# tangle-network/zk-SaaS

Hardware: AMD Instinct MI355X
Metric: Groth16 proofs/sec (SHA-256 circuit) (higher is better)
Workload: dtype u32 limbs (256-bit Montgomery); 1 GPU; BASELINE configs[3]: full distributed Groth16 on the SHA-256 circuit, BN254, l=2, n=8 parties on one GPU, all 12 masks sampled and applied (sha256.rs:226-291); masks=True, constraints=30006, wires=29823, domain=32768, len_a=14911, len_w=14911, len_u=16384, parties=8, packing_factor=2, fixed_base_tables=True

## Files before the change

include/zksaas.h:

```cpp
#ifndef ZKSAAS_H
#define ZKSAAS_H

#include <stddef.h>
#include <stdint.h>

#ifdef __cplusplus
extern "C" {
#endif

typedef struct zk_ctx zk_ctx;

enum zk_curve { ZK_BN254 = 0, ZK_BLS12_381 = 1, ZK_BLS12_377 = 2 };
enum zk_group { ZK_G1 = 1, ZK_G2 = 2 };
enum zk_status { ZK_OK = 0, ZK_ERR_GENERIC = 1, ZK_ERR_PROTOCOL = 2, ZK_ERR_NOT_CONNECTED = 3, ZK_ERR_BAD_INPUT = 4 };

int zk_ctx_create(int curve, int l, int device, zk_ctx** out);
void zk_ctx_destroy(zk_ctx* ctx);
const char* zk_last_error(zk_ctx* ctx, int* party);
int zk_ctx_n(const zk_ctx* ctx);
int zk_ctx_l(const zk_ctx* ctx);
size_t zk_fr_bytes(const zk_ctx* ctx);
size_t zk_fq_bytes(const zk_ctx* ctx);
const char* zk_version(void);

int zk_malloc(zk_ctx* ctx, size_t bytes, void** out_d);
int zk_free(zk_ctx* ctx, void* p_d);
int zk_memcpy_h2d(zk_ctx* ctx, void* dst_d, const void* src, size_t bytes, void* stream);
int zk_memcpy_d2h(zk_ctx* ctx, void* dst, const void* src_d, size_t bytes, void* stream);
int zk_stream_sync(zk_ctx* ctx, void* stream);

void zk_chacha20_block(const uint32_t key[8], uint64_t counter, uint64_t nonce, uint32_t out[16]);

int zk_pss_pack(zk_ctx* ctx, const void* secrets_d, size_t nchunks, int order, uint64_t seed, void* shares_d,
                void* stream);
int zk_pss_det_pack(zk_ctx* ctx, const void* secrets_d, size_t nchunks, int order, void* shares_d,
                    void* stream);
int zk_pss_unpack(zk_ctx* ctx, const void* shares_d, size_t nchunks, void* secrets_d, void* stream);
int zk_pss_unpack2(zk_ctx* ctx, const void* shares_d, const uint32_t* parties, int nparties, size_t nchunks,
                   void* secrets_d, void* stream);

int zk_bitrev(zk_ctx* ctx, void* x_d, int log2_len, void* stream);
int zk_vec_add(zk_ctx* ctx, void* x_d, const void* y_d, size_t len, void* stream);
int zk_vec_scale(zk_ctx* ctx, void* x_d, const void* k, size_t len, void* stream);
int zk_vec_mul_sub(zk_ctx* ctx, void* out_d, const void* a_d, const void* b_d, const void* c_d, size_t len,
                   void* stream);

int zk_fft1(zk_ctx* ctx, void* shares_d, int log2_m, int inverse, size_t batch, const void* add_d, void* stream);
int zk_fq_selftest(zk_ctx* ctx, int op, const void* a_d, const void* b_d, const void* c_d, const void* d_d, size_t len,
                   void* out_d, void* stream);
int zk_fft2_king(zk_ctx* ctx, const void* in_d, const uint32_t* parties, int nparties, int log2_m, int inverse,
                 const void* g, int scale_size_inv, int rearrange, uint64_t seed, void* out_d,
                 const void* out_mask_d, void* stream);
int zk_d_fft(zk_ctx* ctx, void* shares_d, const void* in_mask_d, const void* out_mask_d, int rearrange,
             int log2_m, uint64_t seed, void* out_d, void* stream);
int zk_d_ifft(zk_ctx* ctx, void* shares_d, const void* in_mask_d, const void* out_mask_d, int rearrange,
              int log2_m, const void* g, uint64_t seed, void* out_d, void* stream);
int zk_fft_mask_sample(zk_ctx* ctx, int rearrange, const void* g, int inverse, int log2_m, uint64_t seed,
                       void* in_mask_d, void* out_mask_d, void* stream);

int zk_deg_red(zk_ctx* ctx, void* x_d, const void* in_mask_d, const void* out_mask_d, size_t len, uint64_t seed,
               void* stream);
int zk_deg_red_parties(zk_ctx* ctx, const void* x_d, const uint32_t* parties, int nparties, const void* in_mask_d,
                       const void* out_mask_d, size_t len, uint64_t seed, void* out_d, void* stream);
int zk_degred_mask_sample(zk_ctx* ctx, size_t len, uint64_t seed, void* in_mask_d, void* out_mask_d,
                          void* stream);
int zk_d_pp(zk_ctx* ctx, const void* num_d, const void* den_d, const void* in_mask_d, const void* out_mask_d,
            size_t len, uint64_t seed, void* out_d, void* stream);

int zk_deg_red_points(zk_ctx* ctx, int group, const void* x_d, const void* in_mask_d, const void* out_mask_d, size_t len,
                      const void* gen_affine, uint64_t seed, void* out_d, void* stream);
int zk_degred_mask_sample_points(zk_ctx* ctx, int group, const void* gen_affine, size_t len, uint64_t seed,
                                 void* in_mask_d, void* out_mask_d, void* stream);

int zk_msm(zk_ctx* ctx, int group, const void* bases_d, size_t len_bases, const void* scalars_d,
           size_t len_scalars, void* out, void* stream);
int zk_d_msm(zk_ctx* ctx, int group, const void* bases_d, const void* scalars_d, size_t len, const void* in_mask,
             const void* out_mask, void* out, void* stream);

int zk_pss_pack_points(zk_ctx* ctx, int group, const void* points_d, size_t nchunks, int points_per_chunk,
                       void* shares_d, void* stream);
int zk_base_mul(zk_ctx* ctx, int group, const void* base_affine, const void* scalars_d, size_t len,
                void* out_affine_d, void* stream);

typedef struct zk_groth16_masks {
  const void* fft_in[6];
  const void* fft_out[6];
  const void* degred_in;
  const void* degred_out;
  const void* msm_in[5];
  const void* msm_out[5];
} zk_groth16_masks;

typedef struct zk_crs_share {
  const void* s_d;
  const void* h_d;
  const void* v_d;
  const void* w_d;
  const void* u_d;
  size_t len_a, len_w, len_u;
  const void *a_query0, *b_g1_query0, *delta_g1, *alpha_g1, *beta_g1;
  const void *b_g2_query0, *delta_g2, *beta_g2;
} zk_crs_share;

int zk_circom_h(zk_ctx* ctx, const void* qap_a_d, const void* qap_b_d, const void* qap_c_d, int log2_m,
                const zk_groth16_masks* masks, uint64_t seed, void* h_d, void* stream);
int zk_groth16_prove(zk_ctx* ctx, const zk_crs_share* crs, const void* qap_a_d, const void* qap_b_d,
                     const void* qap_c_d, const void* a_share_d, const void* ax_share_d, const void* r, const void* s,
                     int log2_m, const zk_groth16_masks* masks, uint64_t seed, void* pi_a, void* pi_b, void* pi_c,
                     void* stream);

int zk_d_msm_local(zk_ctx* ctx, int group, const void* bases_d, const void* scalars_d, size_t len, int first_party,
                   int nparties, const void* in_mask, void* out, void* stream);
int zk_group_add(zk_ctx* ctx, int group, const void* a, const void* b, void* out);
int zk_msm_plan(zk_ctx* ctx, int group, size_t len, int plan[4]);
int zk_msm_precompute(zk_ctx* ctx, int group, const void* bases_d, size_t len, void* stream);
int zk_msm_forget(zk_ctx* ctx, const void* bases_d);
int zk_msm_table_info(zk_ctx* ctx, int group, const void* bases_d, int info[2]);
int zk_ctx_set_option(zk_ctx* ctx, const char* name, long long value);
int zk_msm_mask_sample(zk_ctx* ctx, int group, const void* gen_affine, uint64_t seed, void* in_mask, void* out_mask);

int zk_r1cs_qap(zk_ctx* ctx, const void* a_row_ptr_d, const void* a_col_d, const void* a_val_d,
                const void* b_row_ptr_d, const void* b_col_d, const void* b_val_d, const void* w_d,
                size_t num_variables, size_t num_constraints, size_t num_instance, int log_m, void* a_out_d,
                void* b_out_d, void* c_out_d, void* stream);
int zk_fr_to_bytes(zk_ctx* ctx, const void* x_d, size_t len, void* bytes_out_d, void* stream);
int zk_fr_from_bytes(zk_ctx* ctx, const void* bytes_d, size_t len, void* x_out_d, void* stream);
int zk_points_decompress(zk_ctx* ctx, int group, const void* bytes_d, size_t len, void* out_affine_d, void* stream);
int zk_points_compress(zk_ctx* ctx, int group, const void* affine_d, size_t len, void* bytes_out_d, void* stream);
int zk_libsnark_h(zk_ctx* ctx, const void* qap_a_d, const void* qap_b_d, const void* qap_c_d, int log2_m,
                  const void* const* fft_in, const void* const* fft_out, uint64_t seed, void* h_d, void* stream);
int zk_groth16_msms_begin(zk_ctx* ctx, const zk_crs_share* crs, const void* a_share_d, const void* ax_share_d,
                          int first_party, int nparties, int skip_h, const zk_groth16_masks* masks, void* stream);
int zk_groth16_msms_finish(zk_ctx* ctx, const void* h_share_d, void* const* out, void* stream);
int zk_groth16_prove_async(zk_ctx* ctx, const zk_crs_share* crs, const void* qap_a_d, const void* qap_b_d,
                           const void* qap_c_d, const void* a_share_d, const void* ax_share_d, const void* r,
                           const void* s, int log2_m, const zk_groth16_masks* masks, uint64_t seed, void* stream,
                           int* handle);
int zk_groth16_wait(zk_ctx* ctx, int handle, void* pi_a, void* pi_b, void* pi_c);
int zk_groth16_abort(zk_ctx* ctx, int handle);
int zk_groth16_assemble(zk_ctx* ctx, const zk_crs_share* crs, const void* r, const void* s, const void* const* sums,
                        const zk_groth16_masks* masks, void* pi_a, void* pi_b, void* pi_c);
int zk_groth16_prove_batch(zk_ctx* ctx, const zk_crs_share* crs, int nproofs, const void* const* qap_a_d,
                           const void* const* qap_b_d, const void* const* qap_c_d, const void* const* a_share_d,
                           const void* const* ax_share_d, const void* r, const void* s, int log2_m,
                           const zk_groth16_masks* masks, uint64_t seed, void* pi_a, void* pi_b, void* pi_c, void* stream);
int zk_groth16_prove_batch_async(zk_ctx* ctx, const zk_crs_share* crs, int nproofs, const void* const* qap_a_d,
                                 const void* const* qap_b_d, const void* const* qap_c_d, const void* const* a_share_d,
                                 const void* const* ax_share_d, const void* r, const void* s, int log2_m,
                                 const zk_groth16_masks* masks, uint64_t seed, void* stream, int* handle);
int zk_groth16_batch_wait(zk_ctx* ctx, int handle, void* pi_a, void* pi_b, void* pi_c);
int zk_msm_batch(zk_ctx* ctx, int group, const void* bases_d, size_t len, const void* const* scalars_d, int nvec,
                 void* out, void* stream);
int zk_pss_unpack_points(zk_ctx* ctx, int group, const void* shares_d, size_t nchunks, void* out_d, void* stream);
int zk_pss_unpack2_points(zk_ctx* ctx, int group, const void* shares_d, const uint32_t* parties, int nparties,
                          size_t nchunks, void* out_d, void* stream);
int zk_groth16_reconstruct(zk_ctx* ctx, const void* pi_a, const void* pi_b, const void* pi_c, const uint32_t* parties,
                           int nparties, void* proof_affine, void* proof_bytes, void* stream);

typedef struct zk_net zk_net;
enum zk_transport { ZK_NET_LOCAL = 0, ZK_NET_RCCL = 1, ZK_NET_SHM = 2 };
#define ZK_NET_ID_BYTES 512
int zk_net_unique_id(void* id_out);
int zk_net_create(zk_ctx* ctx, int transport, int rank, int world, int n_parties ,
                  const int* party_to_rank, const void* id, size_t shm_bytes_per_channel, zk_net** out);
void zk_net_destroy(zk_net* net);
const char* zk_net_last_error(zk_net* net, int* party);
int zk_net_set_timeout_ms(zk_net* net, uint64_t ms);
int zk_net_info(const zk_net* net, int info[4]);
int zk_net_parties(const zk_net* net, int rank, int* parties );
int zk_net_stats(const zk_net* net, uint64_t stats[4]);
int zk_net_enter(zk_net* net, int sid, uint32_t* mask);
int zk_net_gather(zk_net* net, int sid, uint32_t mask, const void* local, size_t bytes_per_rank, void* full);
int zk_net_scatter(zk_net* net, int sid, uint32_t mask, const void* full, size_t bytes_per_rank, void* local);
int zk_net_alltoall(zk_net* net, int sid, uint32_t mask, const void* send, size_t bytes_per_peer, void* recv);
int zk_net_gather_host(zk_net* net, int sid, uint32_t mask, const void* mine, size_t bytes, void* all);
int zk_net_bcast_host(zk_net* net, int sid, uint32_t mask, void* buf, size_t bytes);
int zk_net_sync(zk_net* net, int sid);

int zk_dist_d_fft(zk_ctx* ctx, zk_net* net, int sid, void* shares_d, const void* in_mask_d, const void* out_mask_d,
                  int rearrange, int log2_m, uint64_t seed, void* stream);
int zk_dist_d_ifft(zk_ctx* ctx, zk_net* net, int sid, void* shares_d, const void* in_mask_d, const void* out_mask_d,
                   int rearrange, int log2_m, const void* g, uint64_t seed, void* stream);
int zk_dist_deg_red(zk_ctx* ctx, zk_net* net, int sid, void* x_d, const void* in_mask_d, const void* out_mask_d,
                    size_t len, uint64_t seed, void* stream);
int zk_dist_d_pp(zk_ctx* ctx, zk_net* net, int sid, const void* num_d, const void* den_d, const void* in_mask_d,
                 const void* out_mask_d, size_t len, uint64_t seed, void* out_d, void* stream);
int zk_dist_d_msm(zk_ctx* ctx, zk_net* net, int sid, int group, const void* bases_d, const void* scalars_d, size_t len,
                  const void* in_mask, const void* out_mask, void* out, void* stream);
int zk_dist_deg_red_points(zk_ctx* ctx, zk_net* net, int sid, int group, const void* x_d, const void* in_mask_d,
                           const void* out_mask_d, size_t len, const void* gen_affine, uint64_t seed, void* out_d,
                           void* stream);
int zk_dist_libsnark_h(zk_ctx* ctx, zk_net* net, const void* qap_a_d, const void* qap_b_d, const void* qap_c_d, int log2_m,
                       const void* const* fft_in_masks, const void* const* fft_out_masks, uint64_t seed, void* h_d,
                       void* stream);
int zk_dist_circom_h(zk_ctx* ctx, zk_net* net, const void* qap_a_d, const void* qap_b_d, const void* qap_c_d, int log2_m,
                     const zk_groth16_masks* masks, uint64_t seed, void* h_d, void* stream);
int zk_dist_groth16_prove(zk_ctx* ctx, zk_net* net, const zk_crs_share* crs, const void* qap_a_d, const void* qap_b_d,
                          const void* qap_c_d, const void* a_share_d, const void* ax_share_d, const void* r, const void* s,
                          int log2_m, const zk_groth16_masks* masks, uint64_t seed, void* pi_a, void* pi_b, void* pi_c,
                          void* stream);

int zk_dist_groth16_prove_async(zk_ctx* ctx, zk_net* net, const zk_crs_share* crs, const void* qap_a_d, const void* qap_b_d,
// ... 41 lines not shown
```

rust/zksaas-hip-sys/src/lib.rs:

```rust
#![allow(non_camel_case_types, non_snake_case, clippy::too_many_arguments)]
use core::ffi::{c_char, c_int, c_long, c_longlong, c_void};

pub const ZK_NET_ID_BYTES: usize = 512;

pub const ZK_BN254: c_int = 0;
pub const ZK_BLS12_381: c_int = 1;
pub const ZK_BLS12_377: c_int = 2;

pub const ZK_G1: c_int = 1;
pub const ZK_G2: c_int = 2;

pub const ZK_OK: c_int = 0;
pub const ZK_ERR_GENERIC: c_int = 1;
pub const ZK_ERR_PROTOCOL: c_int = 2;
pub const ZK_ERR_NOT_CONNECTED: c_int = 3;
pub const ZK_ERR_BAD_INPUT: c_int = 4;

pub const ZK_NET_LOCAL: c_int = 0;
pub const ZK_NET_RCCL: c_int = 1;
pub const ZK_NET_SHM: c_int = 2;

#[repr(C)]
pub struct ZkCtx {
    _private: [u8; 0],
}
#[repr(C)]
pub struct ZkNet {
    _private: [u8; 0],
}

#[repr(C)]
#[derive(Clone, Copy)]
pub struct ZkGroth16Masks {
    pub fft_in: [*const c_void; 6],
    pub fft_out: [*const c_void; 6],
    pub degred_in: *const c_void,
    pub degred_out: *const c_void,
    pub msm_in: [*const c_void; 5],
    pub msm_out: [*const c_void; 5],
}

#[repr(C)]
#[derive(Clone, Copy)]
pub struct ZkCrsShare {
    pub s_d: *const c_void,
    pub h_d: *const c_void,
    pub v_d: *const c_void,
    pub w_d: *const c_void,
    pub u_d: *const c_void,
    pub len_a: usize,
    pub len_w: usize,
    pub len_u: usize,
    pub a_query0: *const c_void,
    pub b_g1_query0: *const c_void,
    pub delta_g1: *const c_void,
    pub alpha_g1: *const c_void,
    pub beta_g1: *const c_void,
    pub b_g2_query0: *const c_void,
    pub delta_g2: *const c_void,
    pub beta_g2: *const c_void,
}

#[link(name = "zksaas_hip")]
extern "C" {
    pub fn zk_ctx_create(curve: c_int, l: c_int, device: c_int, out: *mut *mut ZkCtx) -> c_int;
    pub fn zk_ctx_destroy(ctx: *mut ZkCtx);
    pub fn zk_last_error(ctx: *mut ZkCtx, party: *mut c_int) -> *const c_char;
    pub fn zk_ctx_n(ctx: *const ZkCtx) -> c_int;
    pub fn zk_ctx_l(ctx: *const ZkCtx) -> c_int;
    pub fn zk_fr_bytes(ctx: *const ZkCtx) -> usize;
    pub fn zk_fq_bytes(ctx: *const ZkCtx) -> usize;
    pub fn zk_version() -> *const c_char;
    pub fn zk_malloc(ctx: *mut ZkCtx, bytes: usize, out_d: *mut *mut c_void) -> c_int;
    pub fn zk_free(ctx: *mut ZkCtx, p_d: *mut c_void) -> c_int;
    pub fn zk_memcpy_h2d(
        ctx: *mut ZkCtx,
        dst_d: *mut c_void,
        src: *const c_void,
        bytes: usize,
        stream: *mut c_void,
    ) -> c_int;
    pub fn zk_memcpy_d2h(
        ctx: *mut ZkCtx,
        dst: *mut c_void,
        src_d: *const c_void,
        bytes: usize,
        stream: *mut c_void,
    ) -> c_int;
    pub fn zk_stream_sync(ctx: *mut ZkCtx, stream: *mut c_void) -> c_int;
    pub fn zk_chacha20_block(key: *const u32 , counter: u64, nonce: u64, out: *mut u32 );
    pub fn zk_pss_pack(
        ctx: *mut ZkCtx,
        secrets_d: *const c_void,
        nchunks: usize,
        order: c_int,
        seed: u64,
        shares_d: *mut c_void,
        stream: *mut c_void,
    ) -> c_int;
    pub fn zk_pss_det_pack(
        ctx: *mut ZkCtx,
        secrets_d: *const c_void,
        nchunks: usize,
        order: c_int,
        shares_d: *mut c_void,
        stream: *mut c_void,
    ) -> c_int;
    pub fn zk_pss_unpack(
        ctx: *mut ZkCtx,
        shares_d: *const c_void,
        nchunks: usize,
        secrets_d: *mut c_void,
        stream: *mut c_void,
    ) -> c_int;
    pub fn zk_pss_unpack2(
        ctx: *mut ZkCtx,
        shares_d: *const c_void,
        parties: *const u32,
        nparties: c_int,
        nchunks: usize,
        secrets_d: *mut c_void,
        stream: *mut c_void,
    ) -> c_int;
    pub fn zk_bitrev(ctx: *mut ZkCtx, x_d: *mut c_void, log2_len: c_int, stream: *mut c_void) -> c_int;
    pub fn zk_vec_add(
        ctx: *mut ZkCtx,
        x_d: *mut c_void,
        y_d: *const c_void,
        len: usize,
        stream: *mut c_void,
    ) -> c_int;
    pub fn zk_vec_scale(
        ctx: *mut ZkCtx,
        x_d: *mut c_void,
        k: *const c_void,
        len: usize,
        stream: *mut c_void,
    ) -> c_int;
    pub fn zk_vec_mul_sub(
        ctx: *mut ZkCtx,
        out_d: *mut c_void,
        a_d: *const c_void,
        b_d: *const c_void,
        c_d: *const c_void,
        len: usize,
        stream: *mut c_void,
    ) -> c_int;
    pub fn zk_fft1(
        ctx: *mut ZkCtx,
        shares_d: *mut c_void,
        log2_m: c_int,
        inverse: c_int,
        batch: usize,
        add_d: *const c_void,
        stream: *mut c_void,
    ) -> c_int;
    pub fn zk_fq_selftest(
        ctx: *mut ZkCtx,
        op: c_int,
        a_d: *const c_void,
        b_d: *const c_void,
        c_d: *const c_void,
        d_d: *const c_void,
        len: usize,
        out_d: *mut c_void,
        stream: *mut c_void,
    ) -> c_int;
    pub fn zk_fft2_king(
        ctx: *mut ZkCtx,
        in_d: *const c_void,
        parties: *const u32,
        nparties: c_int,
        log2_m: c_int,
        inverse: c_int,
        g: *const c_void,
        scale_size_inv: c_int,
        rearrange: c_int,
        seed: u64,
        out_d: *mut c_void,
        out_mask_d: *const c_void,
        stream: *mut c_void,
    ) -> c_int;
    pub fn zk_d_fft(
        ctx: *mut ZkCtx,
        shares_d: *mut c_void,
        in_mask_d: *const c_void,
        out_mask_d: *const c_void,
        rearrange: c_int,
        log2_m: c_int,
        seed: u64,
        out_d: *mut c_void,
        stream: *mut c_void,
    ) -> c_int;
    pub fn zk_d_ifft(
        ctx: *mut ZkCtx,
        shares_d: *mut c_void,
        in_mask_d: *const c_void,
        out_mask_d: *const c_void,
        rearrange: c_int,
        log2_m: c_int,
        g: *const c_void,
        seed: u64,
        out_d: *mut c_void,
        stream: *mut c_void,
    ) -> c_int;
    pub fn zk_fft_mask_sample(
        ctx: *mut ZkCtx,
        rearrange: c_int,
        g: *const c_void,
        inverse: c_int,
        log2_m: c_int,
        seed: u64,
        in_mask_d: *mut c_void,
        out_mask_d: *mut c_void,
        stream: *mut c_void,
    ) -> c_int;
    pub fn zk_deg_red(
        ctx: *mut ZkCtx,
        x_d: *mut c_void,
        in_mask_d: *const c_void,
        out_mask_d: *const c_void,
        len: usize,
        seed: u64,
        stream: *mut c_void,
    ) -> c_int;
    pub fn zk_deg_red_parties(
        ctx: *mut ZkCtx,
        x_d: *const c_void,
        parties: *const u32,
        nparties: c_int,
        in_mask_d: *const c_void,
        out_mask_d: *const c_void,
        len: usize,
        seed: u64,
        out_d: *mut c_void,
        stream: *mut c_void,
    ) -> c_int;
    pub fn zk_degred_mask_sample(
        ctx: *mut ZkCtx,
        len: usize,
        seed: u64,
        in_mask_d: *mut c_void,
        out_mask_d: *mut c_void,
        stream: *mut c_void,
    ) -> c_int;
    pub fn zk_d_pp(
        ctx: *mut ZkCtx,
        num_d: *const c_void,
        den_d: *const c_void,
        in_mask_d: *const c_void,
        out_mask_d: *const c_void,
        len: usize,
        seed: u64,
        out_d: *mut c_void,
        stream: *mut c_void,
    ) -> c_int;
    pub fn zk_deg_red_points(
        ctx: *mut ZkCtx,
        group: c_int,
        x_d: *const c_void,
        in_mask_d: *const c_void,
        out_mask_d: *const c_void,
        len: usize,
        gen_affine: *const c_void,
        seed: u64,
        out_d: *mut c_void,
        stream: *mut c_void,
    ) -> c_int;
    pub fn zk_degred_mask_sample_points(
        ctx: *mut ZkCtx,
        group: c_int,
        gen_affine: *const c_void,
        len: usize,
        seed: u64,
        in_mask_d: *mut c_void,
        out_mask_d: *mut c_void,
        stream: *mut c_void,
    ) -> c_int;
    pub fn zk_msm(
        ctx: *mut ZkCtx,
        group: c_int,
        bases_d: *const c_void,
        len_bases: usize,
        scalars_d: *const c_void,
        len_scalars: usize,
        out: *mut c_void,
        stream: *mut c_void,
    ) -> c_int;
    pub fn zk_d_msm(
        ctx: *mut ZkCtx,
        group: c_int,
        bases_d: *const c_void,
        scalars_d: *const c_void,
        len: usize,
        in_mask: *const c_void,
        out_mask: *const c_void,
        out: *mut c_void,
        stream: *mut c_void,
    ) -> c_int;
    pub fn zk_pss_pack_points(
        ctx: *mut ZkCtx,
        group: c_int,
        points_d: *const c_void,
        nchunks: usize,
        points_per_chunk: c_int,
        shares_d: *mut c_void,
        stream: *mut c_void,
    ) -> c_int;
    pub fn zk_base_mul(
        ctx: *mut ZkCtx,
        group: c_int,
        base_affine: *const c_void,
        scalars_d: *const c_void,
        len: usize,
        out_affine_d: *mut c_void,
        stream: *mut c_void,
    ) -> c_int;
    pub fn zk_circom_h(
        ctx: *mut ZkCtx,
        qap_a_d: *const c_void,
// ... 583 lines not shown
```

zk-saas_amd/_lib.py:

```python
import ctypes as C
import os

_HERE = os.path.dirname(os.path.abspath(__file__))
LIB_PATH = os.path.join(_HERE, "libzksaas_hip.so")

SYMBOLS = [
    "zk_version", "zk_ctx_create", "zk_ctx_destroy", "zk_last_error", "zk_ctx_n", "zk_ctx_l", "zk_fr_bytes",
    "zk_fq_bytes", "zk_malloc", "zk_free", "zk_memcpy_h2d", "zk_memcpy_d2h", "zk_stream_sync", "zk_pss_pack",
    "zk_pss_det_pack", "zk_pss_unpack", "zk_pss_unpack2", "zk_bitrev", "zk_vec_add", "zk_vec_mul_sub", "zk_fft1",
    "zk_fft2_king", "zk_d_fft", "zk_d_ifft", "zk_fft_mask_sample", "zk_deg_red", "zk_degred_mask_sample", "zk_d_pp",
    "zk_msm", "zk_d_msm", "zk_base_mul", "zk_circom_h", "zk_groth16_prove", "zk_profile_enable",
    "zk_profile_slots", "zk_profile_name", "zk_profile_read", "zk_d_msm_local", "zk_group_add", "zk_groth16_assemble",
    "zk_groth16_msms_begin", "zk_groth16_msms_finish", "zk_groth16_prove_async", "zk_groth16_wait", "zk_groth16_abort",
    "zk_net_unique_id", "zk_net_create", "zk_net_destroy", "zk_net_last_error", "zk_net_set_timeout_ms", "zk_net_info",
    "zk_net_enter", "zk_net_gather", "zk_net_scatter", "zk_net_alltoall", "zk_net_stats", "zk_net_gather_host", "zk_net_bcast_host", "zk_net_sync",
    "zk_dist_d_fft", "zk_dist_d_ifft", "zk_dist_deg_red", "zk_dist_d_pp", "zk_dist_d_msm", "zk_dist_circom_h",
    "zk_dist_groth16_prove", "zk_chacha20_block", "zk_deg_red_points", "zk_degred_mask_sample_points",
    "zk_points_decompress", "zk_points_compress", "zk_libsnark_h", "zk_vec_scale", "zk_deg_red_parties", "zk_d_msm_parties", "zk_pss_pack_points", "zk_msm_plan",
    "zk_msm_mask_sample", "zk_r1cs_qap", "zk_fr_to_bytes", "zk_fr_from_bytes", "zk_ctx_set_option", "zk_msm_precompute", "zk_msm_forget", "zk_msm_table_info",
    "zk_groth16_prove_batch", "zk_groth16_prove_batch_async", "zk_groth16_batch_wait", "zk_msm_batch", "zk_pss_unpack_points", "zk_pss_unpack2_points", "zk_groth16_reconstruct", "zk_msm_stats", "zk_dist_groth16_prove_batch", "zk_d_fft_host", "zk_msm_host", "zk_d_msm_host",
    "zk_net_parties", "zk_dist_groth16_prove_async", "zk_dist_groth16_wait", "zk_fq_selftest",
    "zk_dist_deg_red_points", "zk_dist_libsnark_h", "zk_deg_red_host", "zk_d_pp_host", "zk_circom_h_host",
    "zk_groth16_prove_host",
]

_lib = None


class ZkError(RuntimeError):

    def __init__(self, code, msg, party=-1):
        super().__init__("zk status %d: %s%s" % (code, msg, (" (party %d)" % party) if party >= 0 else ""))
        self.code, self.msg, self.party = code, msg, party


def _share_hip_runtime_with_torch():
    import importlib.util
    try:
        spec = importlib.util.find_spec("torch")
    except (ImportError, ValueError):
        spec = None
    if spec is None or not spec.origin:
        return
    cand = os.path.join(os.path.dirname(spec.origin), "lib", "libamdhip64.so")
    if os.path.exists(cand):
        try:
            C.CDLL(cand, mode=C.RTLD_GLOBAL)
        except OSError:
            pass


def load():
    global _lib
    if _lib is not None:
        return _lib
    if not os.path.exists(LIB_PATH):
        raise ImportError("libzksaas_hip.so is not built (run `python -c 'import __graft_entry__ as g; g.build()'`); "
                          "there is no CPU fallback")
    os.environ.setdefault("HIP_FORCE_DEV_KERNARG", "1")
    _share_hip_runtime_with_torch()
    lib = C.CDLL(LIB_PATH)
    missing = [name for name in SYMBOLS if not hasattr(lib, name)]
    if missing:
        raise ImportError("%s does not export %s: rebuild it (include/zksaas.h is the ABI)" % (LIB_PATH, ", ".join(missing[:5])))
    vp, sz, u64, i32 = C.c_void_p, C.c_size_t, C.c_uint64, C.c_int
    lib.zk_version.restype = C.c_char_p
    lib.zk_ctx_create.argtypes = [i32, i32, i32, C.POINTER(vp)]
    lib.zk_ctx_destroy.argtypes = [vp]
    lib.zk_ctx_destroy.restype = None
    lib.zk_last_error.argtypes = [vp, C.POINTER(i32)]
    lib.zk_last_error.restype = C.c_char_p
    lib.zk_ctx_n.argtypes = [vp]
    lib.zk_ctx_l.argtypes = [vp]
    lib.zk_fr_bytes.argtypes = [vp]
    lib.zk_fr_bytes.restype = sz
    lib.zk_fq_bytes.argtypes = [vp]
    lib.zk_fq_bytes.restype = sz
    lib.zk_malloc.argtypes = [vp, sz, C.POINTER(vp)]
    lib.zk_free.argtypes = [vp, vp]
    lib.zk_memcpy_h2d.argtypes = [vp, vp, vp, sz, vp]
    lib.zk_memcpy_d2h.argtypes = [vp, vp, vp, sz, vp]
    lib.zk_stream_sync.argtypes = [vp, vp]
    lib.zk_pss_pack.argtypes = [vp, vp, sz, i32, u64, vp, vp]
    lib.zk_pss_det_pack.argtypes = [vp, vp, sz, i32, vp, vp]
    lib.zk_pss_unpack.argtypes = [vp, vp, sz, vp, vp]
    lib.zk_pss_unpack2.argtypes = [vp, vp, C.POINTER(C.c_uint32), i32, sz, vp, vp]
    lib.zk_bitrev.argtypes = [vp, vp, i32, vp]
    lib.zk_vec_add.argtypes = [vp, vp, vp, sz, vp]
    lib.zk_vec_mul_sub.argtypes = [vp, vp, vp, vp, vp, sz, vp]
    lib.zk_fft1.argtypes = [vp, vp, i32, i32, sz, vp, vp]
    lib.zk_fft2_king.argtypes = [vp, vp, C.POINTER(C.c_uint32), i32, i32, i32, vp, i32, i32, u64, vp, vp, vp]
    lib.zk_d_fft.argtypes = [vp, vp, vp, vp, i32, i32, u64, vp, vp]
    lib.zk_d_ifft.argtypes = [vp, vp, vp, vp, i32, i32, vp, u64, vp, vp]
    lib.zk_fft_mask_sample.argtypes = [vp, i32, vp, i32, i32, u64, vp, vp, vp]
    lib.zk_deg_red.argtypes = [vp, vp, vp, vp, sz, u64, vp]
    lib.zk_degred_mask_sample.argtypes = [vp, sz, u64, vp, vp, vp]
    lib.zk_d_pp.argtypes = [vp, vp, vp, vp, vp, sz, u64, vp, vp]
    lib.zk_msm.argtypes = [vp, i32, vp, sz, vp, sz, vp, vp]
    lib.zk_d_msm.argtypes = [vp, i32, vp, vp, sz, vp, vp, vp, vp]
    lib.zk_base_mul.argtypes = [vp, i32, vp, vp, sz, vp, vp]
    lib.zk_circom_h.argtypes = [vp, vp, vp, vp, i32, vp, u64, vp, vp]
    lib.zk_groth16_prove.argtypes = [vp, vp, vp, vp, vp, vp, vp, vp, vp, i32, vp, u64, vp, vp, vp, vp]
    lib.zk_d_msm_local.argtypes = [vp, i32, vp, vp, sz, i32, i32, vp, vp, vp]
    lib.zk_group_add.argtypes = [vp, i32, vp, vp, vp]
    lib.zk_msm_plan.argtypes = [vp, i32, C.c_size_t, C.POINTER(C.c_int)]
    lib.zk_ctx_set_option.argtypes = [vp, C.c_char_p, C.c_longlong]
    lib.zk_msm_precompute.argtypes = [vp, i32, vp, sz, vp]
    lib.zk_msm_forget.argtypes = [vp, vp]
    lib.zk_msm_table_info.argtypes = [vp, i32, vp, C.POINTER(C.c_int)]
    lib.zk_msm_mask_sample.argtypes = [vp, i32, vp, u64, vp, vp]
    lib.zk_r1cs_qap.argtypes = [vp, vp, vp, vp, vp, vp, vp, vp, sz, sz, sz, i32, vp, vp, vp, vp]
    lib.zk_fr_to_bytes.argtypes = [vp, vp, sz, vp, vp]
    lib.zk_fr_from_bytes.argtypes = [vp, vp, sz, vp, vp]
    lib.zk_groth16_assemble.argtypes = [vp, vp, vp, vp, C.POINTER(vp), vp, vp, vp, vp]
    lib.zk_groth16_msms_begin.argtypes = [vp, vp, vp, vp, i32, i32, i32, vp, vp]
    lib.zk_groth16_msms_finish.argtypes = [vp, vp, C.POINTER(vp), vp]
    lib.zk_groth16_prove_async.argtypes = [vp, vp, vp, vp, vp, vp, vp, vp, vp, i32, vp, u64, vp, C.POINTER(i32)]
    lib.zk_groth16_wait.argtypes = [vp, i32, vp, vp, vp]
    lib.zk_groth16_abort.argtypes = [vp, i32]
    u32p = C.POINTER(C.c_uint32)
    lib.zk_chacha20_block.argtypes = [u32p, u64, u64, u32p]
    lib.zk_chacha20_block.restype = None
    lib.zk_deg_red_points.argtypes = [vp, i32, vp, vp, vp, sz, vp, u64, vp, vp]
    lib.zk_degred_mask_sample_points.argtypes = [vp, i32, vp, sz, u64, vp, vp, vp]
    lib.zk_points_decompress.argtypes = [vp, i32, vp, sz, vp, vp]
    lib.zk_points_compress.argtypes = [vp, i32, vp, sz, vp, vp]
    lib.zk_libsnark_h.argtypes = [vp, vp, vp, vp, i32, C.POINTER(vp), C.POINTER(vp), u64, vp, vp]
    lib.zk_net_unique_id.argtypes = [vp]
    lib.zk_net_create.argtypes = [vp, i32, i32, i32, i32, C.POINTER(i32), vp, sz, C.POINTER(vp)]
    lib.zk_net_destroy.argtypes = [vp]
    lib.zk_net_destroy.restype = None
    lib.zk_net_last_error.argtypes = [vp, C.POINTER(i32)]
    lib.zk_net_last_error.restype = C.c_char_p
    lib.zk_net_set_timeout_ms.argtypes = [vp, u64]
    lib.zk_net_info.argtypes = [vp, C.POINTER(i32)]
    lib.zk_net_enter.argtypes = [vp, i32, u32p]
    lib.zk_net_gather.argtypes = [vp, i32, C.c_uint32, vp, sz, vp]
    lib.zk_net_scatter.argtypes = [vp, i32, C.c_uint32, vp, sz, vp]
    lib.zk_net_alltoall.argtypes = [vp, i32, C.c_uint32, vp, sz, vp]
    lib.zk_net_stats.argtypes = [vp, C.POINTER(C.c_uint64)]
    lib.zk_net_gather_host.argtypes = [vp, i32, C.c_uint32, vp, sz, vp]
    lib.zk_net_bcast_host.argtypes = [vp, i32, C.c_uint32, vp, sz]
    lib.zk_net_sync.argtypes = [vp, i32]
    lib.zk_dist_d_fft.argtypes = [vp, vp, i32, vp, vp, vp, i32, i32, u64, vp]
    lib.zk_dist_d_ifft.argtypes = [vp, vp, i32, vp, vp, vp, i32, i32, vp, u64, vp]
    lib.zk_dist_deg_red.argtypes = [vp, vp, i32, vp, vp, vp, sz, u64, vp]
    lib.zk_dist_d_pp.argtypes = [vp, vp, i32, vp, vp, vp, vp, sz, u64, vp, vp]
    lib.zk_dist_d_msm.argtypes = [vp, vp, i32, i32, vp, vp, sz, vp, vp, vp, vp]
    lib.zk_dist_circom_h.argtypes = [vp, vp, vp, vp, vp, i32, vp, u64, vp, vp]
    lib.zk_dist_groth16_prove.argtypes = [vp, vp, vp, vp, vp, vp, vp, vp, vp, vp, i32, vp, u64, vp, vp, vp, vp]
    lib.zk_fq_selftest.argtypes = [vp, i32, vp, vp, vp, vp, sz, vp, vp]
    lib.zk_net_parties.argtypes = [vp, i32, C.POINTER(i32)]
    lib.zk_dist_groth16_prove_async.argtypes = [vp, vp, vp, vp, vp, vp, vp, vp, vp, vp, i32, vp, u64, vp, C.POINTER(i32)]
    lib.zk_dist_groth16_wait.argtypes = [vp, vp, i32, vp, vp, vp]
    lib.zk_dist_groth16_prove_batch.argtypes = [vp, vp, vp, i32, C.POINTER(vp), C.POINTER(vp), C.POINTER(vp), C.POINTER(vp),
                                                C.POINTER(vp), vp, vp, i32, vp, u64, vp, vp, vp, vp]
    lib.zk_d_fft_host.argtypes = [vp, vp, vp, vp, i32, i32, i32, vp, u64, vp]
    lib.zk_deg_red_host.argtypes = [vp, vp, vp, vp, sz, u64, vp]
    lib.zk_d_pp_host.argtypes = [vp, vp, vp, vp, vp, sz, u64, vp, vp]
    lib.zk_circom_h_host.argtypes = [vp, vp, vp, vp, i32, vp, u64, vp, vp]
    lib.zk_groth16_prove_host.argtypes = [vp, vp, vp, vp, vp, vp, vp, vp, vp, i32, vp, u64, vp, vp, vp, vp]
    lib.zk_dist_deg_red_points.argtypes = [vp, vp, i32, i32, vp, vp, vp, sz, vp, u64, vp, vp]
    lib.zk_dist_libsnark_h.argtypes = [vp, vp, vp, vp, vp, i32, C.POINTER(vp), C.POINTER(vp), u64, vp, vp]
    lib.zk_msm_host.argtypes = [vp, i32, vp, sz, vp, sz, vp, vp]
    lib.zk_d_msm_host.argtypes = [vp, i32, vp, vp, sz, vp, vp, vp, vp]
    lib.zk_vec_scale.argtypes = [vp, vp, vp, sz, vp]
    lib.zk_deg_red_parties.argtypes = [vp, vp, C.POINTER(C.c_uint32), i32, vp, vp, sz, u64, vp, vp]
    lib.zk_d_msm_parties.argtypes = [vp, i32, vp, vp, sz, C.POINTER(C.c_uint32), i32, vp, vp, vp, vp]
    lib.zk_pss_pack_points.argtypes = [vp, i32, vp, sz, i32, vp, vp]
    lib.zk_groth16_prove_batch.argtypes = [vp, vp, i32, C.POINTER(vp), C.POINTER(vp), C.POINTER(vp), C.POINTER(vp),
                                           C.POINTER(vp), vp, vp, i32, vp, u64, vp, vp, vp, vp]
    lib.zk_groth16_prove_batch_async.argtypes = [vp, vp, i32, C.POINTER(vp), C.POINTER(vp), C.POINTER(vp), C.POINTER(vp),
                                                 C.POINTER(vp), vp, vp, i32, vp, u64, vp, C.POINTER(i32)]
    lib.zk_groth16_batch_wait.argtypes = [vp, i32, vp, vp, vp]
    lib.zk_msm_batch.argtypes = [vp, i32, vp, sz, C.POINTER(vp), i32, vp, vp]
    lib.zk_pss_unpack_points.argtypes = [vp, i32, vp, sz, vp, vp]
    lib.zk_pss_unpack2_points.argtypes = [vp, i32, vp, C.POINTER(C.c_uint32), i32, sz, vp, vp]
    lib.zk_groth16_reconstruct.argtypes = [vp, vp, vp, vp, C.POINTER(C.c_uint32), i32, vp, vp, vp]
    lib.zk_msm_stats.argtypes = [vp, C.POINTER(C.c_uint64)]
    lib.zk_profile_enable.argtypes = [vp, i32]
    lib.zk_profile_slots.argtypes = []
    lib.zk_profile_name.argtypes = [i32]
    lib.zk_profile_name.restype = C.c_char_p
    lib.zk_profile_read.argtypes = [vp, i32, C.POINTER(C.c_double), C.POINTER(C.c_double), C.POINTER(C.c_long)]
    _lib = lib
    return lib
```

zk-saas_amd/csrc/api.cpp:

```cpp
#include <hip/hip_runtime.h>

#include <cstdlib>
#include <cstring>
#include <new>
#include <string>

#include "../../include/zksaas.h"
#include "engine.hpp"
#include "prng.hpp"

struct zk_ctx {
  zk::IEngine* eng;
};
struct zk_net {
  zk::Net net;
  std::string last;
};

using zk::IEngine;

__attribute__((constructor(101))) static void zk_runtime_defaults() { setenv("HIP_FORCE_DEV_KERNARG", "1", 0); }

static inline hipStream_t S(void* s) { return (hipStream_t)s; }

extern "C" {

const char* zk_version(void) { return "zksaas-hip 0.2 (gfx950)"; }

void zk_chacha20_block(const uint32_t key[8], uint64_t counter, uint64_t nonce, uint32_t out[16]) {
  zk::chacha20_block(key, counter, nonce, out);
}

int zk_ctx_create(int curve, int l, int device, zk_ctx** out) {
  if (!out) return ZK_ERR_BAD_INPUT;
  *out = nullptr;
  int ndev = 0;
  if (hipGetDeviceCount(&ndev) != hipSuccess || ndev <= 0) return ZK_ERR_NOT_CONNECTED;
  if (device < 0 || device >= ndev) return ZK_ERR_BAD_INPUT;
  IEngine* e = nullptr;
  switch (curve) {
    case ZK_BN254: e = zk::make_engine_bn254(l, device); break;
    case ZK_BLS12_381: e = zk::make_engine_bls381(l, device); break;
    case ZK_BLS12_377: e = zk::make_engine_bls377(l, device); break;
    default: return ZK_ERR_BAD_INPUT;
  }
  if (!e) return ZK_ERR_GENERIC;
  zk_ctx* c = new (std::nothrow) zk_ctx{e};
  if (!c) {
    delete e;
    return ZK_ERR_GENERIC;
  }
  *out = c;
  return e->last.code;
}

void zk_ctx_destroy(zk_ctx* ctx) {
  if (!ctx) return;
  delete ctx->eng;
  delete ctx;
}

const char* zk_last_error(zk_ctx* ctx, int* party) {
  if (!ctx) return "null context";
  if (party) *party = ctx->eng->last.party;
  return ctx->eng->last.msg.c_str();
}
int zk_ctx_n(const zk_ctx* ctx) { return ctx ? ctx->eng->n : 0; }
int zk_ctx_l(const zk_ctx* ctx) { return ctx ? ctx->eng->l : 0; }
size_t zk_fr_bytes(const zk_ctx* ctx) { return ctx ? ctx->eng->fr_bytes() : 0; }
size_t zk_fq_bytes(const zk_ctx* ctx) { return ctx ? ctx->eng->fq_bytes() : 0; }

#define CTX_OR_FAIL() \
  if (!ctx) return ZK_ERR_BAD_INPUT; \
  IEngine* e = ctx->eng; \
  (void)hipSetDevice(e->device)

int zk_malloc(zk_ctx* ctx, size_t bytes, void** out_d) {
  CTX_OR_FAIL();
  if (!out_d) return e->fail(ZK_ERR_BAD_INPUT, "null pointer");
  hipError_t h = hipMalloc(out_d, bytes ? bytes : 1);
  return h == hipSuccess ? ZK_OK : e->hip_fail(h, "hipMalloc");
}
int zk_free(zk_ctx* ctx, void* p_d) {
  IEngine* e = ctx ? ctx->eng : nullptr;
  if (e) (void)hipSetDevice(e->device);
  if (p_d) {
    hipDeviceptr_t abase = nullptr;
    size_t asize = 0;
    if (hipMemGetAddressRange(&abase, &asize, (hipDeviceptr_t)p_d) == hipSuccess && asize)
      zk::TableRegistry::inst().forget_range(abase, asize);
    else
      zk::TableRegistry::inst().forget_range(p_d, 1);
  }
  hipError_t h = hipFree(p_d);
  if (h == hipSuccess) return ZK_OK;
  return e ? e->hip_fail(h, "hipFree") : ZK_ERR_GENERIC;
}
int zk_memcpy_h2d(zk_ctx* ctx, void* dst_d, const void* src, size_t bytes, void* stream) {
  CTX_OR_FAIL();
  hipError_t h = hipMemcpyAsync(dst_d, src, bytes, hipMemcpyHostToDevice, S(stream));
  if (h == hipSuccess) h = hipStreamSynchronize(S(stream));
  return h == hipSuccess ? ZK_OK : e->hip_fail(h, "hipMemcpy h2d");
}
int zk_memcpy_d2h(zk_ctx* ctx, void* dst, const void* src_d, size_t bytes, void* stream) {
  CTX_OR_FAIL();
  hipError_t h = hipMemcpyAsync(dst, src_d, bytes, hipMemcpyDeviceToHost, S(stream));
  if (h == hipSuccess) h = hipStreamSynchronize(S(stream));
  return h == hipSuccess ? ZK_OK : e->hip_fail(h, "hipMemcpy d2h");
}
int zk_stream_sync(zk_ctx* ctx, void* stream) {
  CTX_OR_FAIL();
  hipError_t h = hipStreamSynchronize(S(stream));
  return h == hipSuccess ? ZK_OK : e->hip_fail(h, "hipStreamSynchronize");
}

int zk_pss_pack(zk_ctx* ctx, const void* secrets_d, size_t nchunks, int order, uint64_t seed, void* shares_d,
                void* stream) {
  CTX_OR_FAIL();
  return e->pss_pack(secrets_d, nchunks, order, seed, false, shares_d, S(stream));
}
int zk_pss_det_pack(zk_ctx* ctx, const void* secrets_d, size_t nchunks, int order, void* shares_d, void* stream) {
  CTX_OR_FAIL();
  return e->pss_pack(secrets_d, nchunks, order, 0, true, shares_d, S(stream));
}
int zk_pss_unpack(zk_ctx* ctx, const void* shares_d, size_t nchunks, void* secrets_d, void* stream) {
  CTX_OR_FAIL();
  return e->pss_unpack(shares_d, nullptr, e->n, nchunks, false, secrets_d, S(stream));
}
int zk_pss_unpack2(zk_ctx* ctx, const void* shares_d, const uint32_t* parties, int nparties, size_t nchunks,
                   void* secrets_d, void* stream) {
  CTX_OR_FAIL();
  if (!parties && nparties != e->n) return e->fail(ZK_ERR_BAD_INPUT, "parties list required when some are missing");
  return e->pss_unpack(shares_d, parties, nparties, nchunks, true, secrets_d, S(stream));
}

int zk_bitrev(zk_ctx* ctx, void* x_d, int log2_len, void* stream) {
  CTX_OR_FAIL();
  return e->bitrev(x_d, log2_len, S(stream));
}
int zk_vec_add(zk_ctx* ctx, void* x_d, const void* y_d, size_t len, void* stream) {
  CTX_OR_FAIL();
  return e->vec_add(x_d, y_d, len, S(stream));
}
int zk_vec_scale(zk_ctx* ctx, void* x_d, const void* k, size_t len, void* stream) {
  CTX_OR_FAIL();
  return e->vec_scale(x_d, k, len, S(stream));
}
int zk_deg_red_parties(zk_ctx* ctx, const void* x_d, const uint32_t* parties, int nparties, const void* in_mask_d,
                       const void* out_mask_d, size_t len, uint64_t seed, void* out_d, void* stream) {
  CTX_OR_FAIL();
  return e->deg_red_parties(x_d, parties, nparties, in_mask_d, out_mask_d, len, seed, out_d, S(stream));
}
int zk_d_msm_parties(zk_ctx* ctx, int group, const void* bases_d, const void* scalars_d, size_t len,
                     const uint32_t* parties, int nparties, const void* in_mask, const void* out_mask, void* out,
                     void* stream) {
  CTX_OR_FAIL();
  return e->d_msm_parties(group, bases_d, scalars_d, len, parties, nparties, in_mask, out_mask, out, S(stream));
}
int zk_vec_mul_sub(zk_ctx* ctx, void* out_d, const void* a_d, const void* b_d, const void* c_d, size_t len,
                   void* stream) {
  CTX_OR_FAIL();
  return e->vec_mul_sub(out_d, a_d, b_d, c_d, len, S(stream));
}

int zk_fq_selftest(zk_ctx* ctx, int op, const void* a_d, const void* b_d, const void* c_d, const void* d_d, size_t len,
                   void* out_d, void* stream) {
  CTX_OR_FAIL();
  return e->fq_selftest(op, a_d, b_d, c_d, d_d, len, out_d, S(stream));
}

int zk_fft1(zk_ctx* ctx, void* shares_d, int log2_m, int inverse, size_t batch, const void* add_d, void* stream) {
  CTX_OR_FAIL();
  return e->fft1(shares_d, log2_m, inverse, batch, add_d, S(stream));
}
int zk_fft2_king(zk_ctx* ctx, const void* in_d, const uint32_t* parties, int nparties, int log2_m, int inverse,
                 const void* g, int scale_size_inv, int rearrange, uint64_t seed, void* out_d,
                 const void* out_mask_d, void* stream) {
  CTX_OR_FAIL();
  if (!parties && nparties != e->n) return e->fail(ZK_ERR_BAD_INPUT, "parties list required when some are missing");
  if (in_d == out_d) return e->fail(ZK_ERR_BAD_INPUT, "zk_fft2_king cannot run in place (workgroups exchange chunks)");
  return e->fft2_king(in_d, nullptr, parties, nparties, log2_m, inverse, g, scale_size_inv, rearrange, seed, out_d,
                      out_mask_d, S(stream));
}
int zk_d_fft(zk_ctx* ctx, void* shares_d, const void* in_mask_d, const void* out_mask_d, int rearrange, int log2_m,
             uint64_t seed, void* out_d, void* stream) {
  CTX_OR_FAIL();
  return e->d_fft(shares_d, in_mask_d, out_mask_d, rearrange, log2_m, 0, nullptr, seed, out_d, S(stream));
}
int zk_d_ifft(zk_ctx* ctx, void* shares_d, const void* in_mask_d, const void* out_mask_d, int rearrange, int log2_m,
              const void* g, uint64_t seed, void* out_d, void* stream) {
  CTX_OR_FAIL();
  return e->d_fft(shares_d, in_mask_d, out_mask_d, rearrange, log2_m, 1, g, seed, out_d, S(stream));
}
int zk_fft_mask_sample(zk_ctx* ctx, int rearrange, const void* g, int inverse, int log2_m, uint64_t seed,
                       void* in_mask_d, void* out_mask_d, void* stream) {
  CTX_OR_FAIL();
  return e->fft_mask_sample(rearrange, g, inverse, log2_m, seed, in_mask_d, out_mask_d, S(stream));
}

int zk_deg_red(zk_ctx* ctx, void* x_d, const void* in_mask_d, const void* out_mask_d, size_t len, uint64_t seed,
               void* stream) {
  CTX_OR_FAIL();
  return e->deg_red(x_d, in_mask_d, out_mask_d, len, seed, S(stream));
}
int zk_degred_mask_sample(zk_ctx* ctx, size_t len, uint64_t seed, void* in_mask_d, void* out_mask_d, void* stream) {
  CTX_OR_FAIL();
  return e->degred_mask_sample(len, seed, in_mask_d, out_mask_d, S(stream));
}
int zk_d_pp(zk_ctx* ctx, const void* num_d, const void* den_d, const void* in_mask_d, const void* out_mask_d,
            size_t len, uint64_t seed, void* out_d, void* stream) {
  CTX_OR_FAIL();
  return e->d_pp(num_d, den_d, in_mask_d, out_mask_d, len, seed, out_d, S(stream));
}

int zk_msm(zk_ctx* ctx, int group, const void* bases_d, size_t len_bases, const void* scalars_d, size_t len_scalars,
           void* out, void* stream) {
  CTX_OR_FAIL();
  return e->msm(group, bases_d, len_bases, scalars_d, len_scalars, out, S(stream));
}
int zk_d_msm(zk_ctx* ctx, int group, const void* bases_d, const void* scalars_d, size_t len, const void* in_mask,
             const void* out_mask, void* out, void* stream) {
  CTX_OR_FAIL();
  return e->d_msm(group, bases_d, scalars_d, len, in_mask, out_mask, out, S(stream));
}

namespace {
struct HostStage {
  std::vector<void*> bufs;
  ~HostStage() {
    if (!bufs.empty()) (void)hipDeviceSynchronize();
    for (void* p : bufs) (void)hipFree(p);
  }
  void* up(IEngine* e, const void* h, size_t bytes, hipStream_t st, int* rc) {
    void* d = nullptr;
    if (*rc) return nullptr;
    hipError_t he = hipMalloc(&d, bytes ? bytes : 1);
    if (he == hipSuccess) bufs.push_back(d);
    if (he == hipSuccess && h && bytes) he = hipMemcpyAsync(d, h, bytes, hipMemcpyHostToDevice, st);
    if (he != hipSuccess) *rc = e->hip_fail(he, "host staging");
    return d;
  }
};
}
int zk_d_fft_host(zk_ctx* ctx, void* shares , const void* in_mask, const void* out_mask,
                  int rearrange, int log2_m, int inverse, const void* g, uint64_t seed, void* stream) {
  CTX_OR_FAIL();
  if (!shares || log2_m < 0 || log2_m > 40) return e->fail(ZK_ERR_BAD_INPUT, "null pointer");
  const size_t bytes = (size_t)e->n * (((size_t)1 << log2_m) / (size_t)e->l) * e->fr_bytes();
  HostStage hs;
  int rc = ZK_OK;
  void* sd = hs.up(e, shares, bytes, S(stream), &rc);
  void* od = hs.up(e, nullptr, bytes, S(stream), &rc);
  void* im = in_mask ? hs.up(e, in_mask, bytes, S(stream), &rc) : nullptr;
  void* om = out_mask ? hs.up(e, out_mask, bytes, S(stream), &rc) : nullptr;
  if (rc) return rc;
  rc = e->d_fft(sd, im, om, rearrange, log2_m, inverse, g, seed, od, S(stream));
  if (rc) return rc;
  hipError_t he = hipMemcpyAsync(shares, od, bytes, hipMemcpyDeviceToHost, S(stream));
  if (he == hipSuccess) he = hipStreamSynchronize(S(stream));
  return he == hipSuccess ? ZK_OK : e->hip_fail(he, "host staging");
}
int zk_deg_red_host(zk_ctx* ctx, void* x , const void* in_mask, const void* out_mask, size_t len,
                    uint64_t seed, void* stream) {
  CTX_OR_FAIL();
  if (!len) return ZK_OK;
  if (!x) return e->fail(ZK_ERR_BAD_INPUT, "null pointer");
  const size_t bytes = (size_t)e->n * len * e->fr_bytes();
  HostStage hs;
  int rc = ZK_OK;
  void* xd = hs.up(e, x, bytes, S(stream), &rc);
  void* im = in_mask ? hs.up(e, in_mask, bytes, S(stream), &rc) : nullptr;
  void* om = out_mask ? hs.up(e, out_mask, bytes, S(stream), &rc) : nullptr;
  if (rc) return rc;
  rc = e->deg_red(xd, im, om, len, seed, S(stream));
  if (rc) return rc;
  hipError_t he = hipMemcpyAsync(x, xd, bytes, hipMemcpyDeviceToHost, S(stream));
  if (he == hipSuccess) he = hipStreamSynchronize(S(stream));
  return he == hipSuccess ? ZK_OK : e->hip_fail(he, "host staging");
}
int zk_d_pp_host(zk_ctx* ctx, const void* num, const void* den, const void* in_mask, const void* out_mask, size_t len,
                 uint64_t seed, void* out, void* stream) {
  CTX_OR_FAIL();
  if (!len) return ZK_OK;
  if (!num || !den || !out) return e->fail(ZK_ERR_BAD_INPUT, "null pointer");
  const size_t bytes = (size_t)e->n * len * e->fr_bytes();
  HostStage hs;
  int rc = ZK_OK;
  void* nd = hs.up(e, num, bytes, S(stream), &rc);
  void* dd = hs.up(e, den, bytes, S(stream), &rc);
  void* od = hs.up(e, nullptr, bytes, S(stream), &rc);
  void* im = in_mask ? hs.up(e, in_mask, bytes, S(stream), &rc) : nullptr;
  void* om = out_mask ? hs.up(e, out_mask, bytes, S(stream), &rc) : nullptr;
  if (rc) return rc;
  rc = e->d_pp(nd, dd, im, om, len, seed, od, S(stream));
  if (rc) return rc;
  hipError_t he = hipMemcpyAsync(out, od, bytes, hipMemcpyDeviceToHost, S(stream));
  if (he == hipSuccess) he = hipStreamSynchronize(S(stream));
  return he == hipSuccess ? ZK_OK : e->hip_fail(he, "host staging");
}
namespace {
int stage_masks(IEngine* e, HostStage& hs, const zk_groth16_masks* in, size_t bytes, hipStream_t st, zk_groth16_masks* out) {
  int rc = ZK_OK;
  *out = *in;
  for (int i = 0; i < 6; i++) {
    out->fft_in[i] = in->fft_in[i] ? hs.up(e, in->fft_in[i], bytes, st, &rc) : nullptr;
    out->fft_out[i] = in->fft_out[i] ? hs.up(e, in->fft_out[i], bytes, st, &rc) : nullptr;
  }
  out->degred_in = in->degred_in ? hs.up(e, in->degred_in, bytes, st, &rc) : nullptr;
  out->degred_out = in->degred_out ? hs.up(e, in->degred_out, bytes, st, &rc) : nullptr;
  return rc;
}
}
int zk_circom_h_host(zk_ctx* ctx, const void* qap_a, const void* qap_b, const void* qap_c, int log2_m,
                     const zk_groth16_masks* masks, uint64_t seed, void* h, void* stream) {
  CTX_OR_FAIL();
  if (!qap_a || !qap_b || !qap_c || !h || log2_m < 0 || log2_m > 40) return e->fail(ZK_ERR_BAD_INPUT, "null pointer");
  const size_t bytes = (size_t)e->n * (((size_t)1 << log2_m) / (size_t)e->l) * e->fr_bytes();
  HostStage hs;
  int rc = ZK_OK;
  void* a = hs.up(e, qap_a, bytes, S(stream), &rc);
  void* b = hs.up(e, qap_b, bytes, S(stream), &rc);
  void* c = hs.up(e, qap_c, bytes, S(stream), &rc);
// ... 446 lines not shown
```

zk-saas_amd/csrc/engine.hpp:

```cpp
#pragma once
#include <hip/hip_runtime.h>

#include <atomic>
#include <chrono>
#include <map>
#include <memory>
#include <mutex>
#include <string>
#include <thread>
#include <vector>

#include "../../include/zksaas.h"
#include "field.hpp"
#include "ntt.hpp"
#include "pss.hpp"
#include "hostpool.hpp"
#include "net.hpp"

namespace zk {

struct Status {
  int code = ZK_OK;
  int party = -1;
  std::string msg;
// ... 72 lines not shown
  }
  ~ProfScope() {
    if (p) {
      (void)hipEventRecord(b, st);
      p->push({a, b, slot, units});
    }
  }
};

struct MsmTable {
  const char* base = nullptr;
  size_t len = 0, elem = 0;
  int c = 0, nwin = 0, wide = 0, bits = 0, device = 0;
  const void* owner = nullptr;
  void* data = nullptr;
  bool any_identity = true;
  ~MsmTable() {
    if (data) (void)hipFree(data);
  }
};
class TableRegistry {
 public:
  static TableRegistry& inst() {
    static TableRegistry r;
    return r;
  }
  std::shared_ptr<const MsmTable> find(const void* p, size_t npts, size_t elem, int bits, size_t* offset) {
    std::lock_guard<std::mutex> g(mu_);
    const char* q = (const char*)p;
    for (auto& t : v_)
      if (t->elem == elem && t->bits == bits && q >= t->base && q + npts * elem <= t->base + t->len * elem &&
          (size_t)(q - t->base) % elem == 0) {
        *offset = (size_t)(q - t->base) / elem;
        return t;
      }
    return nullptr;
  }
  void add(std::shared_ptr<MsmTable> t) {
    std::lock_guard<std::mutex> g(mu_);
    for (auto& o : v_)
      if (o->base == t->base && o->len == t->len && o->elem == t->elem && o->c == t->c && o->bits == t->bits) return;
    for (auto it = v_.begin(); it != v_.end();)
      if ((*it)->base < t->base + t->len * t->elem && t->base < (*it)->base + (*it)->len * (*it)->elem) it = v_.erase(it);
      else ++it;
    v_.push_back(std::move(t));
  }
  int forget(const void* base) {
    std::lock_guard<std::mutex> g(mu_);
    for (auto it = v_.begin(); it != v_.end(); ++it)
      if ((*it)->base == (const char*)base) {
        v_.erase(it);
        return 1;
      }
    return 0;
  }
  void forget_range(const void* lo_, size_t bytes) {
    std::lock_guard<std::mutex> g(mu_);
    const char* lo = (const char*)lo_;
    for (auto it = v_.begin(); it != v_.end();)
      if ((*it)->base < lo + bytes && lo < (*it)->base + (*it)->len * (*it)->elem) it = v_.erase(it);
      else ++it;
  }
  void forget_owner(const void* owner) {
    std::lock_guard<std::mutex> g(mu_);
    for (auto it = v_.begin(); it != v_.end();)
      if ((*it)->owner == owner) it = v_.erase(it);
      else ++it;
  }

 private:
  std::mutex mu_;
  std::vector<std::shared_ptr<MsmTable>> v_;
};

class IEngine {
 public:
  virtual ~IEngine() {}
  virtual HostPool* host_pool() { return nullptr; }
  std::atomic<int64_t> wait_deadline_ms{120000};
  std::chrono::steady_clock::time_point deadline_from_now() const {
    const int64_t ms = wait_deadline_ms.load(std::memory_order_relaxed);
    return ms > 0 ? std::chrono::steady_clock::now() + std::chrono::milliseconds(ms)
                  : std::chrono::steady_clock::time_point::max();
  }
  hipError_t event_wait(hipEvent_t ev) const {
    using namespace std::chrono;
    hipError_t e = hipEventQuery(ev);
    if (e != hipErrorNotReady) return e;
    const auto t0 = steady_clock::now(), dl = deadline_from_now();
    for (;;) {
      e = hipEventQuery(ev);
      if (e != hipErrorNotReady) return e;
      const auto now = steady_clock::now();
      if (now > dl) return hipErrorNotReady;
      if (now - t0 < milliseconds(2)) std::this_thread::yield();
      else std::this_thread::sleep_for(microseconds(100));
    }
  }
  template <class Pred>
  bool spin_until(Pred ready) const {
    if (ready()) return true;
    const auto dl = deadline_from_now();
    for (unsigned i = 0;; i++) {
      if (ready()) return true;
      std::this_thread::yield();
      if ((i & 1023) == 1023 && std::chrono::steady_clock::now() > dl) return false;
    }
  }
  Profiler prof;
  std::atomic<uint64_t> msm_adds[2] = {{0}, {0}}, msm_offered[2] = {{0}, {0}};
  int l = 0, n = 0, t = 0, device = 0;
  Status last;
  std::mutex last_mu;
  int fail(int code, const std::string& m, int party = -1) {
    std::lock_guard<std::mutex> lk(last_mu);
    last.code = code;
    last.msg = m;
    last.party = party;
    return code;
  }
  int hip_fail(hipError_t e, const char* where) {
    return fail(ZK_ERR_GENERIC, std::string(where) + ": " + hipGetErrorString(e));
  }
  std::atomic<bool> wedged_{false};
  std::string wedged_msg_;
  int wedge(const std::string& what) {
    if (!wedged_.exchange(true)) {
      std::lock_guard<std::mutex> lk(last_mu);
      wedged_msg_ = what;
    }
    return fail(ZK_ERR_GENERIC, what);
  }
  int check_wedged() {
    if (!wedged_.load()) return ZK_OK;
    std::string m;
    {
      std::lock_guard<std::mutex> lk(last_mu);
      m = wedged_msg_;
    }
    return fail(ZK_ERR_GENERIC, "the context is wedged by an earlier timed-out wait (destroy it): " + m);
  }
  virtual size_t fr_bytes() const = 0;
  virtual size_t fq_bytes() const = 0;
  virtual int pss_pack(const void* secrets, size_t nchunks, int order, uint64_t seed, bool det, void* shares,
                       hipStream_t st) = 0;
  virtual int pss_unpack(const void* shares, const uint32_t* parties, int np, size_t nchunks, bool two, void* secrets,
                         hipStream_t st) = 0;
  virtual int bitrev(void* x, int log_len, hipStream_t st) = 0;
  virtual int vec_add(void* x, const void* y, size_t len, hipStream_t st) = 0;
  virtual int vec_scale(void* x, const void* k, size_t len, hipStream_t st) = 0;
  virtual int vec_mul_sub(void* out, const void* a, const void* b, const void* c, size_t len, hipStream_t st) = 0;
  virtual int fq_selftest(int op, const void* a, const void* b, const void* c, const void* d, size_t len, void* out,
                          hipStream_t st) = 0;
  virtual int fft1(void* shares, int log_m, int inverse, size_t batch, const void* add, hipStream_t st) = 0;
  virtual int fft2_king(const void* in, const void* in_mask, const uint32_t* parties, int np, int log_m, int inverse,
                        const void* g, int scale_size_inv, int rearrange, uint64_t seed, void* out,
                        const void* out_mask, hipStream_t st) = 0;
  virtual int d_fft(void* shares, const void* in_mask, const void* out_mask, int rearrange, int log_m, int inverse,
                    const void* g, uint64_t seed, void* out, hipStream_t st) = 0;
  virtual int fft_mask_sample(int rearrange, const void* g, int inverse, int log_m, uint64_t seed, void* in_mask,
                              void* out_mask, hipStream_t st) = 0;
  virtual int deg_red(void* x, const void* in_mask, const void* out_mask, size_t len, uint64_t seed,
                      hipStream_t st) = 0;
  virtual int deg_red_parties(const void* x, const uint32_t* parties, int np, const void* in_mask,
                              const void* out_mask, size_t len, uint64_t seed, void* out, hipStream_t st) = 0;
  virtual int d_msm_parties(int group, const void* bases, const void* scalars, size_t len, const uint32_t* parties,
                            int np, const void* in_mask, const void* out_mask, void* out, hipStream_t st) = 0;
  virtual int degred_mask_sample(size_t len, uint64_t seed, void* in_mask, void* out_mask, hipStream_t st) = 0;
  virtual int d_pp(const void* num, const void* den, const void* in_mask, const void* out_mask, size_t len,
                   uint64_t seed, void* out, hipStream_t st) = 0;
  virtual int msm(int group, const void* bases, size_t nb, const void* scalars, size_t ns, void* out,
                  hipStream_t st) = 0;
  virtual int d_msm(int group, const void* bases, const void* scalars, size_t len, const void* in_mask,
                    const void* out_mask, void* out, hipStream_t st) = 0;
  virtual int d_msm_local(int group, const void* bases, const void* scalars, size_t len, int first_party, int nparties,
                          const void* in_mask, void* out, hipStream_t st) = 0;
  virtual int group_add(int group, const void* a, const void* b, void* out) = 0;
  virtual int msm_plan(int group, size_t len, int* plan) = 0;
  virtual int set_option(const char* name, long long value) = 0;
  virtual int dist_finish(Net* net, int rc) = 0;
  virtual int dist_deg_red_points(Net* net, int sid, int group, const void* x, const void* in_mask, const void* out_mask,
                                  size_t len, const void* gen_affine, uint64_t seed, void* out, hipStream_t st) = 0;
  virtual int dist_libsnark_h(Net* net, const void* qa, const void* qb, const void* qc, int log_m, const void* const* fft_in,
                              const void* const* fft_out, uint64_t seed, void* h, hipStream_t st) = 0;
  virtual int msm_precompute(int group, const void* bases, size_t len, hipStream_t st) = 0;
  virtual int msm_forget(const void* bases) = 0;
  virtual int msm_table_info(int group, const void* bases, int* info) = 0;
  virtual int msm_mask_sample(int group, const void* gen_affine, uint64_t seed, void* in_mask, void* out_mask) = 0;
  virtual int r1cs_qap(const void* pa, const void* ca, const void* va, const void* pb, const void* cb, const void* vb,
                       const void* w, size_t nvars, size_t nc, size_t ni, int log_m, void* a, void* b, void* c,
                       hipStream_t st) = 0;
  virtual int fr_bytes(const void* in, size_t len, void* out, int from_bytes, hipStream_t st) = 0;
  virtual int groth16_assemble(const zk_crs_share* crs, const void* r, const void* s, const void* const* sums,
                               const zk_groth16_masks* masks, void* pi_a, void* pi_b, void* pi_c) = 0;
  virtual int msms_begin(const zk_crs_share* crs, const void* a_share, const void* ax_share, int first, int count,
                         int skip_h, const zk_groth16_masks* masks, hipStream_t st) = 0;
  virtual int msms_finish(const void* h_share, void* const* out, hipStream_t st) = 0;
  virtual int groth16_prove_async(const zk_crs_share* crs, const void* qa, const void* qb, const void* qc,
                                  const void* a_share, const void* ax_share, const void* r, const void* s, int log_m,
                                  const zk_groth16_masks* masks, uint64_t seed, hipStream_t st, int* handle) = 0;
  virtual int groth16_wait(int handle, void* pi_a, void* pi_b, void* pi_c) = 0;
  virtual int groth16_prove_batch(const zk_crs_share* crs, int nb, const void* const* qa, const void* const* qb,
                                  const void* const* qc, const void* const* a_share, const void* const* ax_share,
                                  const void* r, const void* s, int log_m, const zk_groth16_masks* masks, uint64_t seed,
                                  void* pi_a, void* pi_b, void* pi_c, hipStream_t st) = 0;
  virtual int pss_unpack_points(int group, const void* shares, const uint32_t* parties, int np, size_t nchunks, int two,
                                void* out, hipStream_t st) = 0;
  virtual int groth16_reconstruct(const void* pi_a, const void* pi_b, const void* pi_c, const uint32_t* parties, int np,
                                  void* proof_affine, void* proof_bytes, hipStream_t st) = 0;
  virtual int groth16_prove_batch_async(const zk_crs_share* crs, int nb, const void* const* qa, const void* const* qb,
                                        const void* const* qc, const void* const* a_share,
                                        const void* const* ax_share, const void* r, const void* s, int log_m,
                                        const zk_groth16_masks* masks, uint64_t seed, hipStream_t st, int* handle) = 0;
  virtual int groth16_batch_wait(int handle, void* pi_a, void* pi_b, void* pi_c) = 0;
  virtual int msm_batch(int group, const void* bases, size_t len, const void* const* scalars, int nb, void* out,
                        hipStream_t st) = 0;
  virtual int groth16_abort(int handle) = 0;
  virtual int deg_red_points(int group, const void* x, const void* in_mask, const void* out_mask, size_t len,
                             const void* gen_affine, uint64_t seed, void* out, hipStream_t st) = 0;
  virtual int degred_mask_sample_points(int group, const void* gen_affine, size_t len, uint64_t seed, void* in_mask,
                                        void* out_mask, hipStream_t st) = 0;
  virtual int points_codec(int group, const void* in, size_t len, void* out, int decompress, hipStream_t st) = 0;
  virtual int libsnark_h(const void* qa, const void* qb, const void* qc, int log_m, const void* const* fft_in,
                         const void* const* fft_out, uint64_t seed, void* h, hipStream_t st) = 0;
  virtual int dist_d_fft(Net* net, int sid, void* shares, const void* in_mask, const void* out_mask, int rearrange,
                         int log_m, int inverse, const void* g, uint64_t seed, hipStream_t st) = 0;
  virtual int dist_deg_red(Net* net, int sid, void* x, const void* in_mask, const void* out_mask, size_t len,
                           uint64_t seed, hipStream_t st) = 0;
  virtual int dist_d_pp(Net* net, int sid, const void* num, const void* den, const void* in_mask, const void* out_mask,
                        size_t len, uint64_t seed, void* out, hipStream_t st) = 0;
  virtual int dist_d_msm(Net* net, int sid, int group, const void* bases, const void* scalars, size_t len,
                         const void* in_mask, const void* out_mask, void* out, hipStream_t st) = 0;
  virtual int dist_circom_h(Net* net, const void* qa, const void* qb, const void* qc, int log_m,
                            const zk_groth16_masks* masks, uint64_t seed, void* h, hipStream_t st) = 0;
  virtual int dist_prove(Net* net, const zk_crs_share* crs, const void* qa, const void* qb, const void* qc,
                         const void* a_share, const void* ax_share, const void* r, const void* s, int log_m,
                         const zk_groth16_masks* masks, uint64_t seed, void* pi_a, void* pi_b, void* pi_c,
                         hipStream_t st) = 0;
  virtual int dist_prove_async(Net* net, const zk_crs_share* crs, const void* qa, const void* qb, const void* qc,
                               const void* a_share, const void* ax_share, const void* r, const void* s, int log_m,
                               const zk_groth16_masks* masks, uint64_t seed, hipStream_t st, int* handle) = 0;
  virtual int dist_prove_wait(Net* net, int handle, void* pi_a, void* pi_b, void* pi_c) = 0;
  virtual int dist_prove_batch(Net* net, const zk_crs_share* crs, int nb, const void* const* qa, const void* const* qb,
                               const void* const* qc, const void* const* a_share, const void* const* ax_share,
                               const void* r, const void* s, int log_m, const zk_groth16_masks* masks, uint64_t seed,
                               void* pi_a, void* pi_b, void* pi_c, hipStream_t st) = 0;
  virtual int pss_pack_points(int group, const void* points, size_t nchunks, int nv, void* shares, hipStream_t st) = 0;
  virtual int base_mul(int group, const void* base_affine, const void* scalars, size_t len, void* out_affine,
                       hipStream_t st) = 0;
  virtual int circom_h(const void* qa, const void* qb, const void* qc, int log_m, const zk_groth16_masks* masks,
                       uint64_t seed, void* h, hipStream_t st) = 0;
  virtual int groth16_prove(const zk_crs_share* crs, const void* qa, const void* qb, const void* qc,
                            const void* a_share, const void* ax_share, const void* r, const void* s, int log_m,
                            const zk_groth16_masks* masks, uint64_t seed, void* pi_a, void* pi_b, void* pi_c,
                            hipStream_t st) = 0;
};

IEngine* make_engine_bn254(int l, int device);
IEngine* make_engine_bls381(int l, int device);
IEngine* make_engine_bls377(int l, int device);

#define ZK_HIP(expr)                                  \
  do {                                                \
    hipError_t _e = (expr);                           \
    if (_e != hipSuccess) return hip_fail(_e, #expr); \
  } while (0)

inline int ilog2(size_t x) {
  int r = 0;
  while (((size_t)1 << r) < x) r++;
  return r;
}

struct DevBuf {
  void* p = nullptr;
  size_t bytes = 0;
  ~DevBuf() {
    if (p) (void)hipFree(p);
  }
  hipError_t ensure(size_t b) {
    if (b <= bytes) return hipSuccess;
    if (p) (void)hipFree(p);
    p = nullptr;
    bytes = 0;
    hipError_t e = hipMalloc(&p, b);
    if (e == hipSuccess) bytes = b;
    return e;
  }
};

}
```

zk-saas_amd/csrc/engine_fft.inc.hpp:

```cpp

  template <int L>
  int pack_l(const Fr* sec, size_t nch, int order, uint64_t seed, bool det, Fr* shares, hipStream_t st) {
    dim3 grid((unsigned)((nch + KING_THREADS - 1) / KING_THREADS)), block(KING_THREADS);
    if (det)
      pss_pack_kernel<FrP, L, true><<<grid, block, 0, st>>>(sec, nch, order, rs(0), pmat_, pack2_, shares);
    else
      pss_pack_kernel<FrP, L, false><<<grid, block, 0, st>>>(sec, nch, order, rs(seed), pmat_, pack2_, shares);
    ZK_HIP(hipGetLastError());
    return ZK_OK;
  }
  int pss_pack(const void* secrets, size_t nchunks, int order, uint64_t seed, bool det, void* shares,
               hipStream_t st) override {
    if (nchunks == 0) return ZK_OK;
    if (!secrets || !shares) return fail(ZK_ERR_BAD_INPUT, "null pointer");
    const Fr* s = (const Fr*)secrets;
    Fr* o = (Fr*)shares;
    switch (l) {
      case 1: return pack_l<1>(s, nchunks, order, seed, det, o, st);
      case 2: return pack_l<2>(s, nchunks, order, seed, det, o, st);
      case 4: return pack_l<4>(s, nchunks, order, seed, det, o, st);
      default: return pack_l<8>(s, nchunks, order, seed, det, o, st);
    }
  }

  template <int L>
  int unpack_l(const Fr* sh, int np, size_t nch, const Fr* U, Fr* sec, hipStream_t st) {
    dim3 grid((unsigned)((nch + KING_THREADS - 1) / KING_THREADS)), block(KING_THREADS);
    pss_unpack_kernel<FrP, L><<<grid, block, 0, st>>>(sh, np, nch, U, sec);
    ZK_HIP(hipGetLastError());
    return ZK_OK;
  }
  int pss_unpack(const void* shares, const uint32_t* parties, int np, size_t nchunks, bool two, void* secrets,
                 hipStream_t st) override {
    if (nchunks == 0) return ZK_OK;
    if (!secrets || !shares) return fail(ZK_ERR_BAD_INPUT, "null pointer");
    const Fr* U = nullptr;
    if (!two) {
      if (np != n) return fail(ZK_ERR_BAD_INPUT, "unpack needs all n shares");
      U = umats_[key_u(0xffffffffu, 1)];
    } else {
      int rc = umat_for(parties, np, &U);
      if (rc) return rc;
    }
    const Fr* s = (const Fr*)shares;
    Fr* o = (Fr*)secrets;
    switch (l) {
      case 1: return unpack_l<1>(s, np, nchunks, U, o, st);
      case 2: return unpack_l<2>(s, np, nchunks, U, o, st);
      case 4: return unpack_l<4>(s, np, nchunks, U, o, st);
      default: return unpack_l<8>(s, np, nchunks, U, o, st);
    }
  }

  int bitrev(void* x, int log_len, hipStream_t st) override {
    if (log_len < 0 || log_len > 40) return fail(ZK_ERR_BAD_INPUT, "bad length");
    size_t len = (size_t)1 << log_len;
    bitrev_kernel<Fr><<<dim3((unsigned)((len + 255) / 256)), dim3(256), 0, st>>>((Fr*)x, log_len);
    ZK_HIP(hipGetLastError());
    return ZK_OK;
  }
  int vec_add(void* x, const void* y, size_t len, hipStream_t st) override {
    if (!len) return ZK_OK;
    vec_add_kernel<Fr><<<dim3((unsigned)((len + 255) / 256)), dim3(256), 0, st>>>((Fr*)x, (const Fr*)y, len);
    ZK_HIP(hipGetLastError());
    return ZK_OK;
  }
  int vec_scale(void* x, const void* k, size_t len, hipStream_t st) override {
    if (!len) return ZK_OK;
    if (!x || !k) return fail(ZK_ERR_BAD_INPUT, "null pointer");
    vec_scale_kernel<Fr><<<dim3((unsigned)((len + 255) / 256)), dim3(256), 0, st>>>((Fr*)x, Fr::from_limbs((const uint32_t*)k),
                                                                                 len);
    ZK_HIP(hipGetLastError());
    return ZK_OK;
  }
  int vec_mul_sub(void* out, const void* a, const void* b, const void* c, size_t len, hipStream_t st) override {
    if (!len) return ZK_OK;
    const unsigned bk = (unsigned)king_block(len);
    size_t wgs = (len + bk - 1) / bk;
    if (bk == 64 && wgs > 512) wgs = 512;
    vec_mul_sub_kernel<Fr><<<dim3((unsigned)wgs), dim3(bk), 0, st>>>((Fr*)out, (const Fr*)a, (const Fr*)b, (const Fr*)c, len);
    ZK_HIP(hipGetLastError());
    return ZK_OK;
  }

  int fq_selftest(int op, const void* a, const void* b, const void* c, const void* d, size_t len, void* out,
                  hipStream_t st) override {
    using Fq = Fp<typename Cfg::FqP>;
    if (!len) return ZK_OK;
    if (!a || !b || !c || !d || !out) return fail(ZK_ERR_BAD_INPUT, "null pointer");
    if (op < 0 || op > 17) return fail(ZK_ERR_BAD_INPUT, "op must be 0 .. 17");
    if (op >= 2 && !Fq::LAZY_OK) return fail(ZK_ERR_BAD_INPUT, "this base field has no lazy form");
    if (op == 1 && !Cfg::HAS_G2) return fail(ZK_ERR_BAD_INPUT, "G2 is not available for this curve");
    fq_selftest_kernel<Fq, (Fq::N == 8)><<<dim3((unsigned)((len + 255) / 256)), dim3(256), 0, st>>>(
        op, (const Fq*)a, (const Fq*)b, (const Fq*)c, (const Fq*)d, len, (Fq*)out);
    ZK_HIP(hipGetLastError());
    return ZK_OK;
  }

  int fft1(void* shares, int log_m, int inverse, size_t batch, const void* add, hipStream_t st) override {
    return fft1_src(shares, log_m, inverse, batch, add, st, NttSrc<Fr>{{nullptr, nullptr, nullptr}, 1});
  }
  int fft1_src(void* shares, int log_m, int inverse, size_t batch, const void* add, hipStream_t st, NttSrc<Fr> src) {
    int log_l = ilog2(l);
    if (log_m < log_l) return fail(ZK_ERR_BAD_INPUT, "Mismatch of size in FFT");
    int log_n = log_m - log_l;
    if (batch == 0) return ZK_OK;
    const Fr* tw = nullptr;
    int rc = gentab(log_m, inverse, st, &tw);
    if (rc) return rc;
    Fr* data = (Fr*)shares;
    size_t nvec = (size_t)1 << log_n;
    if (log_n < NTT_TILE_BITS_SMALL && src.p[0]) {
      for (size_t y = 0; y < batch; y += src.per)
        ZK_HIP(hipMemcpyAsync(data + y * nvec, src.p[y / src.per], (size_t)src.per * nvec * sizeof(Fr),
                              hipMemcpyDeviceToDevice, st));
    }
    if (log_n < NTT_TILE_BITS_SMALL) {
      for (int s = 1; s <= log_n; s++) {
        size_t work = (nvec / 2) * batch;
        ntt_stage_simple_kernel<Fr><<<dim3((unsigned)((work + 255) / 256)), dim3(256), 0, st>>>(data, log_n, s, tw,
                                                                                                log_l, batch);
        ZK_HIP(hipGetLastError());
      }
      if (add) return vec_add(shares, add, nvec * batch, st);
      return ZK_OK;
    }
    if (ntt_tile_bits(log_n) == NTT_TILE_BITS_SMALL && (small_groups() || log_n < NTT_TILE_BITS))
      return fft1_tiled<NTT_TILE_BITS_SMALL>(data, log_n, log_l, batch, tw, (const Fr*)add, st, src);
    return fft1_tiled<NTT_TILE_BITS>(data, log_n, log_l, batch, tw, (const Fr*)add, st, src);
  }
  template <int TB>
  int fft1_tiled(Fr* data, int log_n, int log_l, size_t batch, const Fr* tw, const Fr* add, hipStream_t st,
                 NttSrc<Fr> src) {
    constexpr size_t TILE = (size_t)1 << TB;
    const size_t nvec = (size_t)1 << log_n;
    NttPlan plan = make_ntt_plan(log_n, TB);
    if (plan.npass == 0) return fail(ZK_ERR_BAD_INPUT, "transform too large for the four-pass plan");
    for (int p = 0; p < plan.npass; p++) {
      const NttPass& ps = plan.pass[p];
      int rbits = ps.s1 - ps.s0;
      const int tws = (TB >= 10 && rbits >= 4) ? 2 : 0;
      const int tws_eff = rbits >= 4 ? tws : 0;
      size_t lds = (size_t)(sizeof(Fr) / 16) * 16 * (TILE + ((((size_t)1 << rbits) / 2) >> tws_eff) + 1);
      bool& attr_set = ntt_attr_set_[TB == NTT_TILE_BITS_SMALL ? 0 : 1];
      if (!attr_set) {
        ZK_HIP(hipFuncSetAttribute((const void*)ntt_pass_kernel<Fr, TB>, hipFuncAttributeMaxDynamicSharedMemorySize,
                                   (int)((sizeof(Fr) / 16) * 16 * (TILE + TILE / 2 + 1))));
        attr_set = true;
      }
      dim3 grid((unsigned)(nvec >> TB), (unsigned)batch);
      ProfScope ps_(prof, PROF_NTT_PASS, st, (double)nvec * batch);
      ntt_pass_kernel<Fr, TB><<<grid, dim3((unsigned)(TILE / 4)), lds, st>>>(
          data, log_n, ps.s0, ps.s1, ps.cbits, tw, log_l, p == plan.npass - 1 ? add : nullptr,
          p == 0 ? src : NttSrc<Fr>{{nullptr, nullptr, nullptr}, 1}, tws_eff);
      ZK_HIP(hipGetLastError());
    }
    return ZK_OK;
  }

  template <int L>
  int king_l(const Fr* in, const KingBatch<Fr>& kb, int batch, int np, int log_lc, const Fr* U, const Fr* gen,
             const GTab* gt, const Fr* in_scale, int rearrange, uint64_t seed_, Fr* out, bool negate, hipStream_t st,
             const KingRange* range = nullptr) {
    size_t Lc = (size_t)1 << log_lc;
    const size_t kbk = (size_t)king_block(Lc);
    size_t Wc = Lc < kbk ? Lc : kbk;
    size_t lds = (size_t)L * Wc * sizeof(Fr);
    const size_t cols = range ? range->cnt : Lc;
    if (range && (Wc == Lc || range->rs % Wc || range->seg % Wc || range->cnt % Wc || batch != 1))
      return fail(ZK_ERR_GENERIC, "bad king range");
    if (!cols) return ZK_OK;
    dim3 grid((unsigned)(cols / Wc), (unsigned)batch), block((unsigned)kbk);
    ProfScope ps_(prof, PROF_KING, st, (double)cols * batch);
    const RngSeed seed = rs(seed_, kb.seed_off((uint32_t)batch - 1) + 1);
    const uint32_t rs_ = range ? range->rs : 0u, seg_ = range ? range->seg : 0u;
    if (negate)
      king_fft2_kernel<FrP, L, true><<<grid, block, lds, st>>>(in, kb, np, (uint32_t)log_lc, U, pmat_, gen,
                                                               gt ? gt->tab : nullptr, gt ? gt->step : nullptr,
                                                               in_scale, pack2_, rearrange, seed, out, rs_, seg_);
    else
      king_fft2_kernel<FrP, L, false><<<grid, block, lds, st>>>(in, kb, np, (uint32_t)log_lc, U, pmat_, gen,
                                                                gt ? gt->tab : nullptr, gt ? gt->step : nullptr,
                                                                in_scale, pack2_, rearrange, seed, out, rs_, seg_);
    ZK_HIP(hipGetLastError());
    return ZK_OK;
  }
  int king_dispatch_batch(const Fr* in, const KingBatch<Fr>& kb, int batch, int np, int log_m, int inverse,
                          const Fr* U, const void* g, int scale, int rearrange, uint64_t seed, Fr* out, bool negate,
                          hipStream_t st, const KingRange* range = nullptr) {
    int log_l = ilog2(l);
    if (log_m < log_l) return fail(ZK_ERR_BAD_INPUT, "Mismatch of size in FFT");
    if (batch < 1 || batch > KING_BATCH) return fail(ZK_ERR_BAD_INPUT, "bad king batch");
    const bool has_in_mask = kb.in_mask[0] != nullptr;
    for (int y = 1; y < batch; y++)
      if ((kb.in_mask[y] != nullptr) != has_in_mask) return fail(ZK_ERR_BAD_INPUT, "mixed in-masks in one batch");
    const Fr* gen = nullptr;
    int rc = gentab(log_m, inverse, st, &gen);
    if (rc) return rc;
    Fr gv = g ? Fr::from_limbs((const uint32_t*)g) : Fr::one();
    GTab gt{};
    bool fold = scale && !has_in_mask;
    const Fr* in_scale = nullptr;
    if (scale && has_in_mask) {
      rc = size_inv_dev(log_m, st, &in_scale);
      if (rc) return rc;
    }
    bool need = fold || gv != Fr::one();
    if (need) {
      rc = gtab(log_m, gv, fold, st, &gt);
      if (rc) return rc;
    }
    int log_lc = log_m - log_l;
    switch (l) {
      case 1: return king_l<1>(in, kb, batch, np, log_lc, U, gen, need ? &gt : nullptr, in_scale, rearrange, seed, out, negate, st, range);
      case 2: return king_l<2>(in, kb, batch, np, log_lc, U, gen, need ? &gt : nullptr, in_scale, rearrange, seed, out, negate, st, range);
      case 4: return king_l<4>(in, kb, batch, np, log_lc, U, gen, need ? &gt : nullptr, in_scale, rearrange, seed, out, negate, st, range);
      default: return king_l<8>(in, kb, batch, np, log_lc, U, gen, need ? &gt : nullptr, in_scale, rearrange, seed, out, negate, st, range);
    }
  }
  int king_dispatch(const Fr* in, const Fr* in_mask, int np, int log_m, int inverse, const Fr* U, const void* g,
                    int scale, int rearrange, uint64_t seed, Fr* out, const Fr* out_mask, bool negate,
                    hipStream_t st, const KingRange* range = nullptr) {
    KingBatch<Fr> kb{};
    kb.in_mask[0] = in_mask;
    kb.out_mask[0] = out_mask;
    kb.stride = 0;
    return king_dispatch_batch(in, kb, 1, np, log_m, inverse, U, g, scale, rearrange, seed, out, negate, st, range);
  }
  int fft2_king(const void* in, const void* in_mask, const uint32_t* parties, int np, int log_m, int inverse,
                const void* g, int scale_size_inv, int rearrange, uint64_t seed, void* out, const void* out_mask,
                hipStream_t st) override {
    if (!in || !out) return fail(ZK_ERR_BAD_INPUT, "null pointer");
    const Fr* U = nullptr;
    int rc = umat_for(parties, np, &U);
    if (rc) return rc;
    return king_dispatch((const Fr*)in, (const Fr*)in_mask, np, log_m, inverse, U, g, scale_size_inv, rearrange, seed,
                         (Fr*)out, (const Fr*)out_mask, false, st);
  }

  int d_fft(void* shares, const void* in_mask, const void* out_mask, int rearrange, int log_m, int inverse,
            const void* g, uint64_t seed, void* out, hipStream_t st) override {
    if (!shares) return fail(ZK_ERR_BAD_INPUT, "null pointer");
    if (out == shares) out = nullptr;
    int log_l = ilog2(l);
    if (log_m < log_l) return fail(ZK_ERR_BAD_INPUT, "Mismatch of size in FFT");
    size_t bytes = (size_t)n * (((size_t)1 << log_m) / l) * sizeof(Fr);
    DevBuf& king_tmp_ = ws(st)->king_tmp;
    ZK_HIP(king_tmp_.ensure(bytes));
    NttSrc<Fr> src{};
// ... 187 lines not shown
```

zk-saas_amd/csrc/msm.hpp:

```cpp
#pragma once
#include <algorithm>
#include <atomic>
#include <cstdio>
#include <cstdlib>
#include <future>
#include <map>
#include <memory>
#include <mutex>
#include <type_traits>
#include <vector>

#include "ec.hpp"
#include "engine.hpp"
#include "msm_plan.hpp"
#include "ntt.hpp"
#include "quad.hpp"

namespace zk {
#if defined(__HIPCC__)

enum MsmRole { ROLE_SH, ROLE_W, ROLE_V, ROLE_U, NROLES };
constexpr const char* ROLE_NAME[NROLES] = {"S+H", "W", "V", "U"};
constexpr int NJOBS = 2;
constexpr int NBATCH = 3;
// ... 836 lines not shown
    uint32_t end_k = offsets[k + 1];
    const bool skip_pt = pt.is_identity();
    const bool was_id = acc.is_identity();
    Fld U2 = Fld::zero(), S2 = Fld::zero();
    {
      const Fld y2 = (e_cur >> 31) ? pt.y.neg() : pt.y;
      if (!skip_pt) {
        if (was_id) {
          acc = XYZZ<Fld>{pt.x, y2, Fld::one(), Fld::one()};
        } else if constexpr (acc_lazy_v<Fld>) {
          U2 = Fld::mul_lazy(pt.x, acc.ZZ);
          S2 = Fld::mul_lazy(y2, acc.ZZZ);
        } else {
          U2 = pt.x * acc.ZZ;
          S2 = y2 * acc.ZZZ;
        }
      }
    }
    e = e1;
    pt = load_elem(bases + (e & 0x7fffffffu));
    e1 = sorted[p + 2 < b ? p + 2 : b - 1];
    if constexpr (acc_lazy_v<Fld>) {
      if (!skip_pt && !was_id) {
        const Fld P = Fld::sub_lazy(U2, acc.X);
        const Fld R = Fld::sub_lazy(S2, acc.Y);
        if (P.is_zero_lazy()) {
          if (R.is_zero_lazy()) {
            const Affine<Fld> q = load_elem(bases + (e_cur & 0x7fffffffu));
            acc = xyzz_dbl_affine(q.x, (e_cur >> 31) ? q.y.neg() : q.y);
          } else {
            acc = XYZZ<Fld>::identity();
          }
        } else {
          const Fld PP = Fld::mul_lazy(P, P);
          const Fld PPP = Fld::mul_lazy(P, PP);
          const Fld Q = Fld::mul_lazy(acc.X, PP);
          const Fld X3 = Fld::sub_lazy(Fld::sub_lazy(Fld::mul_lazy(R, R), PPP), Fld::dbl_lazy(Q));
          const Fld Y3 = Fld::mul_sub_mul_lazy(R, Fld::sub_lazy(Q, X3), acc.Y, PPP);
          acc = XYZZ<Fld>{X3, Y3, Fld::mul_lazy(acc.ZZ, PP), Fld::mul_lazy(acc.ZZZ, PPP)};
        }
      }
    } else if (!skip_pt && !was_id) {
      const Fld P = U2 - acc.X;
      const Fld R = S2 - acc.Y;
      if (P.is_zero()) {
        if (R.is_zero()) {
          const Affine<Fld> q = load_elem(bases + (e_cur & 0x7fffffffu));
          acc = xyzz_dbl_affine(q.x, (e_cur >> 31) ? q.y.neg() : q.y);
        } else {
          acc = XYZZ<Fld>::identity();
        }
      } else {
        const Fld PP = P.sqr();
        const Fld PPP = P * PP;
        const Fld Q = acc.X * PP;
        const Fld X3 = R.sqr() - PPP - Q.dbl();
        const Fld Y3 = Fld::mul_sub_mul(R, Q - X3, acc.Y, PPP);
        acc = XYZZ<Fld>{X3, Y3, acc.ZZ * PP, acc.ZZZ * PPP};
      }
    }
    while (end_k <= p) {
      k++;
      end_k = offsets[k + 1];
    }
    if (p + 1 == end_k || p + 1 == b) {
      XYZZ<Fld>* dst = cont ? head + lane : (p + 1 == end_k ? buckets + k : tail + lane);
      if constexpr (acc_lazy_v<Fld>) acc = XYZZ<Fld>{acc.X.canon(), acc.Y.canon(), acc.ZZ.canon(), acc.ZZZ.canon()};
      store_elem_untracked(dst, acc);
      if (!cont && p + 1 != end_k && (blockIdx.y == 0 || ys != 0) && (end_k - 1) / T - lane > FIN_SEQ)
        msm_report_heavy(heavy, k, (end_k - 1) / T - lane);
      acc = XYZZ<Fld>::identity();
      cont = false;
      k += p + 1 == end_k ? 1u : 0u;
    }
  }
}

template <class P>
constexpr int SPLIT_WAVES = P::N > 8 ? 3 : 4;
template <class P>
__global__ __launch_bounds__(128, SPLIT_WAVES<P>) void msm_accumulate_split_kernel(const void* __restrict__ bases0,
                                                                 const void* __restrict__ bases1,
                                                                 const uint32_t* __restrict__ sorted,
                                                                 const uint32_t* __restrict__ offsets, uint32_t nkeys,
                                                                 uint32_t nlanes, uint32_t tmin, uint32_t cap,
                                                                 void* __restrict__ buckets0, void* __restrict__ edge0,
                                                                 uint32_t* __restrict__ heavy,
                                                                 const uint32_t* __restrict__ k0, size_t ys) {
  using F = Fp<P>;
  constexpr size_t AFF = 4, SUM = 8;
  ZK_YSHIFT(sorted);
  ZK_YSHIFT(offsets);
  ZK_YSHIFT(heavy);
  ZK_YSHIFT(k0);
  const F* __restrict__ bases = reinterpret_cast<const F*>(blockIdx.y ? bases1 : bases0);
  F* __restrict__ buckets = reinterpret_cast<F*>(buckets0) + (size_t)blockIdx.y * nkeys * SUM;
  F* __restrict__ head = reinterpret_cast<F*>(edge0) + (size_t)blockIdx.y * 2 * nlanes * SUM;
  F* __restrict__ tail = head + (size_t)nlanes * SUM;
  const uint32_t total = offsets[nkeys];
  const uint32_t T = msm_range_len(total, nlanes, tmin, cap);
  const uint32_t q = threadIdx.x & 3;
  const bool comp = (q & 1) != 0, half = (q & 2) != 0;
  const uint32_t lane = blockIdx.x * (blockDim.x / 4) + (threadIdx.x >> 2);
  if (lane >= nlanes || (uint64_t)lane * T >= total) return;
  const uint32_t a = lane * T, b = a + T < total ? a + T : total;
  uint32_t k = k0[lane];
  bool cont = offsets[k] < a;
  uint32_t end_k = offsets[k + 1];
  uint32_t end_n = offsets[k + 2 <= nkeys ? k + 2 : nkeys];
  SplitAcc<P> acc = split_identity<P>(comp);
  uint32_t e = sorted[a];
  uint32_t e1 = a + 1 < b ? sorted[a + 1] : e;
  F pt = load_elem(bases + (size_t)(e & 0x7fffffffu) * AFF + q);
  for (uint32_t p = a; p < b; p++) {
    const uint32_t e_next = e1;
    if (p + 2 < b) e1 = sorted[p + 2];
    F pt_next = pt;
    if (p + 1 < b) pt_next = load_elem(bases + (size_t)(e_next & 0x7fffffffu) * AFF + q);
    uint32_t z = pt.is_zero() ? 1u : 0u;
    z &= qperm_u32<1, 0, 3, 2>(z);
    z &= qperm_u32<2, 3, 0, 1>(z);
    if (!z) {
      const F c = qsel(half && (e >> 31) != 0, pt.neg(), pt);
      acc = split_madd<P>(acc, c, half, comp);
    }
    if (p + 1 == end_k || p + 1 == b) {
      F* dst = cont ? head + (size_t)lane * SUM : (p + 1 == end_k ? buckets + (size_t)k * SUM : tail + (size_t)lane * SUM);
      store_elem(dst + q, acc.c0);
      store_elem(dst + 4 + q, acc.c1);
      if (q == 0 && !cont && p + 1 != end_k && (blockIdx.y == 0 || ys != 0) && (end_k - 1) / T - lane > FIN_SEQ)
        msm_report_heavy(heavy, k, (end_k - 1) / T - lane);
      acc = split_identity<P>(comp);
      cont = false;
      if (p + 1 < b) {
        k++;
        end_k = end_n;
        while (end_k == p + 1) {
          k++;
          end_k = offsets[k + 1];
        }
        end_n = offsets[k + 2 <= nkeys ? k + 2 : nkeys];
      }
    }
    e = e_next;
    pt = pt_next;
  }
}

constexpr int QUAD_THREADS = 256;
constexpr int QUAD_VL = QUAD_THREADS / 4;
inline int quad_threads(bool batched) {
  return batched ? 64 : 256;
}

template <class Fld>
__global__ __launch_bounds__(64) void msm_heavy_kernel(const XYZZ<Fld>* __restrict__ edge0, uint32_t nlanes, uint32_t tmin,
                                                       uint32_t cap, const uint32_t* __restrict__ offsets, uint32_t nkeys,
                                                       XYZZ<Fld>* __restrict__ buckets0,
                                                       const uint32_t* __restrict__ heavy,
                                                       XYZZ<Fld>* __restrict__ hpart0, uint32_t vcap, size_t ys) {
  __builtin_amdgcn_s_setprio(3);
  ZK_YSHIFT(offsets);
  ZK_YSHIFT(heavy);
  const uint32_t nh = heavy[1], V = heavy[0];
  if (blockIdx.x >= V) return;
  const XYZZ<Fld>* __restrict__ head = edge0 + (size_t)blockIdx.y * 2 * nlanes;
  const XYZZ<Fld>* __restrict__ tail = head + nlanes;
  XYZZ<Fld>* __restrict__ buckets = buckets0 + (size_t)blockIdx.y * nkeys;
  XYZZ<Fld>* __restrict__ hpart = hpart0 + (size_t)blockIdx.y * vcap;
  extern __shared__ uint4 smem_fin[];
  XYZZ<Fld>* sh = reinterpret_cast<XYZZ<Fld>*>(smem_fin);
  const uint32_t T = msm_range_len(offsets[nkeys], nlanes, tmin, cap);
  const int q = threadIdx.x & 3, vl = threadIdx.x >> 2;
  const int nq = (int)blockDim.x / 4;
  for (uint32_t v = blockIdx.x; v < V; v += gridDim.x) {
    uint32_t lo = 0, hi = nh;
    while (hi - lo > 1) {
      const uint32_t mid = (lo + hi) >> 1;
      if (heavy[3 + 2 * mid] <= v) lo = mid;
      else hi = mid;
    }
    const uint32_t kh = heavy[2 + 2 * lo], vb = heavy[3 + 2 * lo];
    const uint32_t S = (lo + 1 < nh ? heavy[3 + 2 * (lo + 1)] : V) - vb, s = v - vb;
    const uint32_t o0 = offsets[kh], o1 = offsets[kh + 1];
    const uint32_t l0 = o0 / T, l1 = (o1 - 1) / T;
    const uint32_t chunk = (l1 - l0 + S - 1) / S;
    const uint32_t first = l0 + 1 + s * chunk, last = first + chunk - 1 < l1 ? first + chunk - 1 : l1;
    Fld acc = (s == 0 && vl == 0) ? qload(tail + l0, q) : qidentity<Fld>(q);
    for (uint32_t l = first + (uint32_t)vl; l <= last; l += (uint32_t)nq) acc = qadd(acc, qload(head + l, q), q);
    acc = wg_quad_sum(acc, sh, vl, q, nq);
    if (vl == 0) qstore(S == 1 ? buckets + kh : hpart + v, q, acc);
    __syncthreads();
  }
}

constexpr int FIN_THREADS = 64;
template <class Fld>
__global__ __launch_bounds__(FIN_THREADS) void msm_finalize_kernel(const XYZZ<Fld>* __restrict__ edge0, uint32_t nlanes,
                                                               uint32_t tmin, uint32_t cap,
                                                               const uint32_t* __restrict__ offsets, uint32_t nkeys,
                                                               XYZZ<Fld>* __restrict__ buckets0,
                                                               const uint32_t* __restrict__ heavy,
                                                               const XYZZ<Fld>* __restrict__ hpart0, uint32_t vcap,
                                                               uint32_t fin_wgs, size_t ys) {
  __builtin_amdgcn_s_setprio(3);
  ZK_YSHIFT(offsets);
  const XYZZ<Fld>* __restrict__ head = edge0 + (size_t)blockIdx.y * 2 * nlanes;
  const XYZZ<Fld>* __restrict__ tail = head + nlanes;
  XYZZ<Fld>* __restrict__ buckets = buckets0 + (size_t)blockIdx.y * nkeys;
  const int q = threadIdx.x & 3;
  if (blockIdx.x >= fin_wgs) {
    ZK_YSHIFT(heavy);
    const uint32_t nh = heavy[1], V = heavy[0];
    const XYZZ<Fld>* __restrict__ hpart = hpart0 + (size_t)blockIdx.y * vcap;
    extern __shared__ uint4 smem_fin[];
    XYZZ<Fld>* sh = reinterpret_cast<XYZZ<Fld>*>(smem_fin);
    const int vl = threadIdx.x >> 2;
    for (uint32_t h = blockIdx.x - fin_wgs; h < nh; h += gridDim.x - fin_wgs) {
      const uint32_t vb = heavy[3 + 2 * h], S = (h + 1 < nh ? heavy[3 + 2 * (h + 1)] : V) - vb;
      if (S == 1) continue;
      Fld acc = qidentity<Fld>(q);
      for (uint32_t j = (uint32_t)vl; j < S; j += FIN_THREADS / 4) acc = qadd(acc, qload(hpart + vb + j, q), q);
      acc = wg_quad_sum(acc, sh, vl, q, FIN_THREADS / 4);
      if (vl == 0) qstore(buckets + heavy[2 + 2 * h], q, acc);
      __syncthreads();
    }
    return;
  }
  const uint32_t T = msm_range_len(offsets[nkeys], nlanes, tmin, cap);
  for (size_t k = (size_t)blockIdx.x * (FIN_THREADS / 4) + (threadIdx.x >> 2); k < nkeys;
       k += (size_t)fin_wgs * (FIN_THREADS / 4)) {
    const uint32_t o0 = offsets[k], o1 = offsets[k + 1];
    if (o0 == o1) {
      qstore(buckets + k, q, qidentity<Fld>(q));
      continue;
    }
    const uint32_t l0 = o0 / T, l1 = (o1 - 1) / T;
    if (l1 == l0 || l1 - l0 > FIN_SEQ) continue;
    Fld acc = qload(tail + l0, q);
    for (uint32_t l = l0 + 1; l <= l1; l++) acc = qadd(acc, qload(head + l, q), q);
    qstore(buckets + k, q, acc);
  }
}

template <class Fld>
__global__ __launch_bounds__(QUAD_THREADS, 2) void msm_reduce_a_kernel(const XYZZ<Fld>* __restrict__ buckets0, uint32_t B,
                                                                   int lo_bits, int nvl, XYZZ<Fld>* __restrict__ out0) {
  __builtin_amdgcn_s_setprio(3);
  extern __shared__ uint4 smem_red[];
  XYZZ<Fld>* sh = reinterpret_cast<XYZZ<Fld>*>(smem_red);
  const uint32_t LO = 1u << lo_bits, HI = B >> lo_bits;
  const uint32_t ngroups = HI + 1 + LO;
  const XYZZ<Fld>* __restrict__ wb = buckets0 + (size_t)blockIdx.y * B;
  const int q = threadIdx.x & 3, vl = threadIdx.x >> 2;
  const uint32_t g = blockIdx.x * (uint32_t)((int)blockDim.x / 4 / nvl) + (uint32_t)(vl / nvl);
  const uint32_t sub = (uint32_t)(vl & (nvl - 1));
  Fld acc = qidentity<Fld>(q);
  if (g <= HI) {
    for (uint32_t lo = sub; lo < LO; lo += (uint32_t)nvl) {
      uint32_t k = g * LO + lo;
      if (k >= 1 && k <= B) acc = qadd(acc, qload(wb + (k - 1), q), q);
    }
  } else if (g < ngroups) {
    const uint32_t lo = g - HI - 1;
    for (uint32_t hi = sub; hi <= HI; hi += (uint32_t)nvl) {
      uint32_t k = hi * LO + lo;
      if (k >= 1 && k <= B) acc = qadd(acc, qload(wb + (k - 1), q), q);
    }
  }
  acc = wg_quad_sum(acc, sh, vl, q, nvl);
  if (sub == 0 && g < ngroups) qstore(out0 + (size_t)blockIdx.y * ngroups + g, q, acc);
}

template <class Fld>
__global__ __launch_bounds__(QUAD_THREADS, 2) void msm_reduce_b_kernel(const XYZZ<Fld>* __restrict__ rc0, uint32_t B, int lo_bits,
                                                                   int nvl, XYZZ<Fld>* __restrict__ out0,
                                                                   const uint32_t* __restrict__ cnt_src, size_t cnt_stride,
                                                                   uint32_t ncnt, uint32_t* __restrict__ cnt_dst) {
  __builtin_amdgcn_s_setprio(3);
  if (blockIdx.x == 0 && blockIdx.y == 0 && threadIdx.x < ncnt)
    cnt_dst[2 * threadIdx.x] = *(const uint32_t*)((const char*)cnt_src + threadIdx.x * cnt_stride);
  extern __shared__ uint4 smem_red[];
  XYZZ<Fld>* sh = reinterpret_cast<XYZZ<Fld>*>(smem_red);
  const uint32_t LO = 1u << lo_bits, HI = B >> lo_bits;
  const uint32_t ngroups = HI + 1 + LO;
  int hb = 0;
  while ((1u << hb) < HI) hb++;
  const int nslices = hb + 1 + lo_bits;
  const XYZZ<Fld>* __restrict__ rc = rc0 + (size_t)blockIdx.y * ngroups;
  const int q = threadIdx.x & 3, vl = threadIdx.x >> 2;
  const int j = (int)blockIdx.x * ((int)blockDim.x / 4 / nvl) + vl / nvl;
  const uint32_t sub = (uint32_t)(vl & (nvl - 1));
  Fld acc = qidentity<Fld>(q);
  if (j <= hb) {
    for (uint32_t hi = sub; hi <= HI; hi += (uint32_t)nvl)
      if ((hi >> j) & 1u) acc = qadd(acc, qload(rc + hi, q), q);
  } else if (j < nslices) {
    const int jj = j - hb - 1;
    for (uint32_t lo = sub; lo < LO; lo += (uint32_t)nvl)
      if ((lo >> jj) & 1u) acc = qadd(acc, qload(rc + HI + 1 + lo, q), q);
  }
  acc = wg_quad_sum(acc, sh, vl, q, nvl);
  if (sub == 0 && j < nslices) qstore(out0 + (size_t)blockIdx.y * nslices + j, q, acc);
}

template <class Fld>
__global__ __launch_bounds__(128) void msm_table_kernel(const Affine<Fld>* __restrict__ bases, size_t len, int c,
                                                       int nwin, int wide, Affine<Fld>* __restrict__ table) {
  size_t i = (size_t)blockIdx.x * blockDim.x + threadIdx.x;
  if (i >= len) return;
  Affine<Fld> p = load_elem(bases + i);
  if (p.is_identity()) {
    for (int w = 0; w < nwin; w++) store_elem(table + (size_t)w * len + i, p);
    return;
  }
  XYZZ<Fld> acc = XYZZ<Fld>::from_affine(p);
  int left = 0;
  for (int w = 0; w < nwin;) {
    if (left == 0) {
      store_elem(table + (size_t)w * len + i, xyzz_to_affine(acc));
      left = w < wide ? c : c - 1;
      w++;
      if (w == nwin) break;
    }
    acc = xyzz_dbl(acc);
    left--;
  }
}

#endif

template <class Fld>
struct KernelField {
  using type = Fld;
};
template <class P>
struct KernelField<Fp2T<P, false>> {
  using type = Fp2T<P, (P::N <= ZK_MUL_INLINE_LIMBS)>;
};

struct MsmSlot {
  DevBuf ws;
  void* pinned = nullptr;
  size_t pinned_bytes = 0;
  hipEvent_t ev = nullptr;
  std::atomic<bool> busy{false};
  std::shared_ptr<const MsmTable> tab, tab2;
  hipError_t wait(const IEngine* eng) {
    if (!busy) return hipSuccess;
    hipError_t he = eng->event_wait(ev);
    if (he == hipErrorNotReady) return he;
    tab.reset();
    tab2.reset();
    busy = false;
    return he;
  }
  ~MsmSlot() {
    if (pinned) (void)hipHostFree(pinned);
    if (ev) (void)hipEventDestroy(ev);
  }
  hipError_t ensure_pinned(size_t b) {
    if (b <= pinned_bytes) return hipSuccess;
    if (pinned) (void)hipHostFree(pinned);
    pinned = nullptr;
    pinned_bytes = 0;
    hipError_t e = hipHostMalloc(&pinned, b, hipHostMallocDefault);
    if (e == hipSuccess) pinned_bytes = b;
    return e;
  }
};

struct MsmBatchArg {
  int nb = 1;
  const void* p[16] = {nullptr};
};

struct MsmPending {
  MsmFoldGeo fold;
  MsmSlot* slot = nullptr;
};

struct MsmGate {
  hipEvent_t sorted_ev = nullptr;
  std::atomic<int>* sorted_cnt = nullptr;
  const hipEvent_t* wait_sorted = nullptr;
  int n_wait_sorted = 0, sorted_need = 0;
  hipEvent_t wait_ev = nullptr;
  std::atomic<int>* wait_flag = nullptr;
  hipEvent_t signal_ev = nullptr;
  std::atomic<int>* signal_flag = nullptr;
};

struct MsmTuning {
  size_t bigsort_min;
  MsmGate gate;
  int c_force = 0;
};

template <class FrP, class Fld>
int msm_launch(IEngine* eng, MsmSlot& slot, const MsmTuning& tune, const void* bases, const void* bases2,
               const void* scalars, size_t npts, const Fp<FrP>* coef_d, size_t part_len, hipStream_t st,
               MsmPending* out, const MsmBatchArg* batch = nullptr);
template <class FrP, class Fld>
int pack_points_split_launch(IEngine* eng, const void* points, size_t nchunks, int n, const uint8_t* dig, int jlen,
                             const void* beta , void* shares, hipStream_t st);
template <class FrP, class Fld>
int base_mul_split_launch(IEngine* eng, const void* scalars, size_t len, const void* table, int nwin, int wb, void* out,
                          hipStream_t st);
template <class FrP, class Fld>
int msm_table_launch(IEngine* eng, const void* bases, size_t len, int c, int nwin, int wide, void* table,
                     hipStream_t st);

template <class Fld>
int msm_fold_batch(IEngine* eng, MsmPending& p, XYZZ<Fld>* results, int nvec) {
  const MsmFoldGeo& f = p.fold;
  const int batch = f.batch;
  for (int i = 0; i < nvec * batch; i++) results[i] = XYZZ<Fld>::identity();
  if (!p.slot) return ZK_OK;
  hipError_t he = p.slot->wait(eng);
  if (he == hipErrorNotReady)
    return eng->fail(ZK_ERR_GENERIC, std::string("msm fold: the completion event of a ") + (f.g2 ? "G2" : "G1") +
                                         " MSM chain did not signal within the deadline (zk_ctx_set_option wait_deadline_ms)");
  if (he != hipSuccess) return eng->hip_fail(he, "msm event");
  const int kwin = f.kwin, lo_bits = f.lo_bits, nslices = f.win.c;
  const int hb = f.win.c - 1 - lo_bits;
  const XYZZ<Fld>* hall = (const XYZZ<Fld>*)p.slot->pinned;
  {
    const uint32_t* cnt = (const uint32_t*)((const char*)p.slot->pinned + f.stats_off);
    uint64_t adds = 0;
    for (int v = 0; v < f.nb; v++) adds += cnt[2 * (f.nsorts == 2 ? v : 0)];
    eng->msm_adds[f.g2 ? 1 : 0].fetch_add(adds, std::memory_order_relaxed);
    eng->msm_offered[f.g2 ? 1 : 0].fetch_add(f.offered, std::memory_order_relaxed);
  }
  if (nvec > f.nb) nvec = f.nb;
  auto fold_range = [&](const XYZZ<Fld>* h, int w_hi, int w_lo) -> XYZZ<Fld> {
    XYZZ<Fld> total = XYZZ<Fld>::identity();
    for (int w = w_hi; w >= w_lo; w--) {
      const XYZZ<Fld>* sl = h + (size_t)w * nslices;
      for (int t = f.win.width(w) - 1; t >= 0; t--) {
        total = xyzz_dbl_ni(total);
        const XYZZ<Fld>& s = t >= lo_bits ? sl[t - lo_bits] : sl[hb + 1 + t];
        if (!s.is_identity()) total = xyzz_add_ni(total, s);
      }
    }
    return total;
  };
  constexpr int FOLD_PARTS_MAX = 8;
  HostPool* pool = eng->host_pool();
  auto sets_of = [&](int v, int b) { return hall + ((size_t)v * batch + b) * kwin * nslices; };
  if (batch > 1) {
    const int jobs = nvec * batch;
    if (kwin > 1 && pool && pool->idle() >= jobs) {
      std::vector<std::future<void>> futs;
      for (int i = 1; i < jobs; i++) {
        XYZZ<Fld>* dst = results + i;
        const XYZZ<Fld>* h = sets_of(i / batch, i % batch);
        futs.push_back(pool->submit([=, &fold_range]() { *dst = fold_range(h, kwin - 1, 0); }));
      }
      results[0] = fold_range(sets_of(0, 0), kwin - 1, 0);
      for (auto& f : futs)
        while (!pool->wait_helping(f, eng->deadline_from_now())) {}
    } else {
      for (int i = 0; i < jobs; i++) results[i] = fold_range(sets_of(i / batch, i % batch), kwin - 1, 0);
    }
    return ZK_OK;
  }
  const int max_parts = !pool ? 1 : std::min({FOLD_PARTS_MAX, kwin / 2, (pool->idle() + 1) / std::max(nvec, 1)});
  if (max_parts < 2) {
    for (int v = 0; v < nvec; v++) results[v] = fold_range(sets_of(v, 0), kwin - 1, 0);
    return ZK_OK;
  }
  std::vector<int> start(kwin + 1, 0);
  for (int w = 0; w <= kwin; w++) start[w] = f.win.start(w);
  constexpr double ADD_COST = 0.6;
  auto partition = [&](double bound, int* hi_w, int* lo_w) {
    int np = 0, w = kwin - 1;
    while (w >= 0) {
      if (np == FOLD_PARTS_MAX) return FOLD_PARTS_MAX + 1;
      hi_w[np] = w;
      double cost = start[w + 1] + ADD_COST * nslices;
      w--;
      while (w >= 0 && cost + ADD_COST * nslices <= bound) cost += ADD_COST * nslices, w--;
      lo_w[np++] = w + 1;
    }
    return np;
  };
  int hi_w[FOLD_PARTS_MAX], lo_w[FOLD_PARTS_MAX];
  double lo_b = start[kwin] + ADD_COST * nslices, hi_b = start[kwin] + ADD_COST * nslices * kwin;
  for (int it = 0; it < 24; it++) {
    const double mid = 0.5 * (lo_b + hi_b);
    if (partition(mid, hi_w, lo_w) <= max_parts) hi_b = mid;
    else lo_b = mid;
  }
  const int nparts = partition(hi_b, hi_w, lo_w);
  auto fold_part = [&fold_range, &start](const XYZZ<Fld>* h, int w_hi, int w_lo) {
    XYZZ<Fld> t = fold_range(h, w_hi, w_lo);
    if (!t.is_identity())
      for (int i = 0; i < start[w_lo]; i++) t = xyzz_dbl_ni(t);
    return t;
  };
  XYZZ<Fld> part[2][FOLD_PARTS_MAX];
  std::vector<std::future<void>> futs;
  for (int v = 0; v < nvec; v++)
    for (int g = 0; g < nparts; g++) {
      if (v == 0 && g == 0) continue;
      const XYZZ<Fld>* h = sets_of(v, 0);
      XYZZ<Fld>* dst = &part[v][g];
      const int a = hi_w[g], b = lo_w[g];
      futs.push_back(pool->submit([=, &fold_part]() { *dst = fold_part(h, a, b); }));
    }
  part[0][0] = fold_part(hall, hi_w[0], lo_w[0]);
  for (auto& f : futs)
    while (!pool->wait_helping(f, eng->deadline_from_now())) {}
  for (int v = 0; v < nvec; v++) {
    XYZZ<Fld> total = part[v][0];
    for (int g = 1; g < nparts; g++) total = xyzz_add_ni(total, part[v][g]);
    results[v] = total;
  }
  return ZK_OK;
}

template <class Fld>
int msm_fold(IEngine* eng, MsmPending& p, XYZZ<Fld>* result, XYZZ<Fld>* result2) {
  if (p.slot && p.fold.batch != 1) return eng->fail(ZK_ERR_GENERIC, "msm_fold on a batched launch");
  XYZZ<Fld> r[2];
  int rc = msm_fold_batch<Fld>(eng, p, r, result2 ? 2 : 1);
  *result = r[0];
  if (result2) *result2 = r[1];
  return rc;
}

template <class FrP, class Fld>
inline XYZZ<Fld> host_straus(const XYZZ<Fld>* pts, const Fp<FrP>* k_mont, int np) {
  std::vector<XYZZ<Fld>> tab((size_t)np * 15);
  std::vector<Fp<FrP>> k((size_t)np);
  for (int p = 0; p < np; p++) {
    k[p] = k_mont[p].from_mont();
    tab[(size_t)p * 15] = pts[p];
    for (int d = 1; d < 15; d++)
      tab[(size_t)p * 15 + d] = (d & 1) ? xyzz_dbl_ni(tab[(size_t)p * 15 + d / 2])
                                        : xyzz_add_ni(tab[(size_t)p * 15 + d - 1], pts[p]);
  }
  XYZZ<Fld> acc = XYZZ<Fld>::identity();
  for (int nib = FrP::N * 8 - 1; nib >= 0; nib--) {
    for (int i = 0; i < 4; i++) acc = xyzz_dbl_ni(acc);
    for (int p = 0; p < np; p++) {
      uint32_t d = (k[p].v[nib / 8] >> (4 * (nib % 8))) & 15u;
      if (d) acc = xyzz_add_ni(acc, tab[(size_t)p * 15 + d - 1]);
    }
  }
  return acc;
}

template <class Cfg>
class MsmRunner {
 public:
  using FrP = typename Cfg::FrP;
  using Fr = Fp<FrP>;
  using Fq = Fp<typename Cfg::FqP>;
  using Fq2 = Fp2<typename Cfg::FqP>;

// ... 221 lines not shown
```

zk-saas_amd/csrc/msm_impl.hpp:

```cpp
#pragma once
#include "msm.hpp"
#include "pack_split.hpp"

namespace zk {

#define MSM_HIP(x)                                           \
  do {                                                       \
    hipError_t _e = (x);                                     \
    if (_e != hipSuccess) return eng->hip_fail(_e, #x);      \
  } while (0)
#ifdef ZK_MSM_DEBUG_SYNC
#define MSM_STAGE(name)                                                          \
  do {                                                                           \
    hipError_t _e = hipStreamSynchronize(st);                                    \
    fprintf(stderr, "[zk msm] %s done (%s) npts=%zu c=%d nwin=%d\n", name,       \
            hipGetErrorString(_e), pl.npts, pl.win.c, pl.win.nwin);              \
    if (_e != hipSuccess) return eng->hip_fail(_e, name);                        \
  } while (0)
#else
#define MSM_STAGE(name) do { } while (0)
#endif

template <class Fr, class KF>
struct MsmViews {
  uint32_t *counts, *heavy, *bins, *cursor, *offsets, *bt, *sorted, *k0, *tmp, *zero;
  uint16_t *tmp_lo, *tcnt;
  Fr* canon;
  XYZZ<KF>*edge, *buckets, *hpart, *rc;
  XYZZ<KF>* out;
  uint32_t* stats;
  MsmViews(const MsmPlan& pl, void* ws, void* pinned) {
    auto at = [&](MsmRegionId id) { return (char*)ws + pl.r[id].off; };
    counts = (uint32_t*)at(R_COUNTS), heavy = (uint32_t*)at(R_HEAVY), bins = (uint32_t*)at(R_BINS);
    cursor = (uint32_t*)at(R_CURSOR), offsets = (uint32_t*)at(R_OFFSETS), bt = (uint32_t*)at(R_BT);
    sorted = (uint32_t*)at(R_SORTED), k0 = (uint32_t*)at(R_K0), tmp = (uint32_t*)at(R_TMP);
    zero = (uint32_t*)((char*)ws + pl.zero_off);
    tmp_lo = (uint16_t*)at(R_TMP_LO), tcnt = pl.use_tcnt ? (uint16_t*)at(R_TCNT) : nullptr;
    canon = (Fr*)at(R_CANON);
    edge = (XYZZ<KF>*)at(R_EDGE), buckets = (XYZZ<KF>*)at(R_BUCKETS), hpart = (XYZZ<KF>*)at(R_HPART), rc = (XYZZ<KF>*)at(R_RC);
    out = (XYZZ<KF>*)pinned, stats = (uint32_t*)((char*)pinned + pl.out_bytes);
  }
};

template <class... P, class... A>
hipError_t msm_launch_lds(int device, void (*kernel)(P...), dim3 grid, dim3 block, size_t lds, hipStream_t st, A... args) {
  if (lds > 48 * 1024) {
    hipError_t e = msm_lds_attr((const void*)kernel, lds, device);
    if (e != hipSuccess) return e;
  }
  kernel<<<grid, block, lds, st>>>(args...);
  return hipSuccess;
}

template <class FrP, class KF>
int msm_stage_sort(IEngine* eng, const MsmPlan& pl, const MsmViews<Fp<FrP>, KF>& v, const MsmScalars<Fp<FrP>>& sc,
                   const Fp<FrP>* coef_d, size_t plen, const MsmBaseId& bid, hipStream_t st) {
  const size_t npts = pl.npts, ys = pl.ys, nkeys = pl.nkeys;
  const unsigned batch = (unsigned)pl.batch, NS = pl.nsorts;
  const int c = pl.win.c, nwin = pl.win.nwin, wide = pl.win.wide, sort_hi = pl.sort_hi, sort_lo = pl.sort_lo;
  MSM_HIP(msm_zero(v.zero, pl.zero_bytes, st, NS, ys));
  auto tiles = [&](size_t tile_pts) { return (unsigned)((npts + tile_pts - 1) / tile_pts); };
  ProfScope ps_(eng->prof, PROF_MSM_SORT, st, (double)npts * batch);
  if (pl.big) {
    const uint32_t wmask = pl.tabbed ? 0u : ~0u;
    const bool wf = pl.wide_fmt;
    {
      const unsigned tpv = tiles((size_t)BIG_THREADS * pl.hist_ppt);
      MSM_HIP(msm_launch_lds(eng->device, msm_hist_kernel<FrP>, dim3(tpv * batch, NS), dim3(BIG_THREADS), pl.hist_lds, st,
                             sc, coef_d, plen, c, nwin, wide, sort_hi, sort_lo, pl.hist_ppt, tpv, wmask, v.bins, bid, v.canon,
                             v.tcnt, ys));
    }
    if (pl.large) {
      const unsigned tpv = tiles(pl.tile_pts);
      auto* k = wf ? msm_scatter_kernel<FrP, 1024, BIG_PTS_PER_THREAD, true> : msm_scatter_kernel<FrP, 1024, BIG_PTS_PER_THREAD, false>;
      switch (pl.ppt) {
        case BIG_PTS_PER_THREAD: break;
        case 4: k = wf ? msm_scatter_kernel<FrP, 1024, 4, true> : msm_scatter_kernel<FrP, 1024, 4, false>; break;
        case 2: k = wf ? msm_scatter_kernel<FrP, 1024, 2, true> : msm_scatter_kernel<FrP, 1024, 2, false>; break;
        case 1: k = wf ? msm_scatter_kernel<FrP, 1024, 1, true> : msm_scatter_kernel<FrP, 1024, 1, false>; break;
        default: return eng->fail(ZK_ERR_GENERIC, "msm: unsupported scatter tile");
      }
      MSM_HIP(msm_launch_lds(eng->device, k, dim3(tpv * batch, NS), dim3(1024), pl.scatter_lds, st, sc, c, nwin, wide, sort_hi,
                             sort_lo, tpv, wmask, pl.wgroup, pl.pre_stride, pl.pre_off, pl.idx_bits, (uint32_t)pl.stage_cap,
                             v.bins, v.tmp, v.tmp_lo, v.canon, v.tcnt, ys));
    } else {
      const unsigned tpv = tiles((size_t)BIG_THREADS * pl.ppt);
      MSM_HIP(msm_launch_lds(eng->device, wf ? msm_scatter_direct_kernel<FrP, true> : msm_scatter_direct_kernel<FrP, false>,
                             dim3(tpv * batch, NS), dim3(BIG_THREADS), pl.scatter_lds, st, sc, c, nwin, wide, sort_hi, sort_lo,
                             pl.ppt, tpv, wmask, pl.pre_stride, pl.pre_off, pl.idx_bits, v.bins, v.tmp, v.tmp_lo, v.canon, ys));
    }
    auto* bk = pl.large ? (wf ? msm_binsort_kernel<1024, true, true> : msm_binsort_kernel<1024, false, true>)
                        : (wf ? msm_binsort_kernel<256, true, false> : msm_binsort_kernel<256, false, false>);
    MSM_HIP(msm_launch_lds(eng->device, bk, dim3((unsigned)pl.nbins_tot, NS), dim3((unsigned)pl.sthr), pl.binsort_lds, st, v.tmp,
                           v.tmp_lo, v.bins, (uint32_t)pl.nbins_tot, sort_hi, sort_lo, (uint32_t)(c - 1), pl.idx_bits,
                           (uint32_t)nkeys, pl.nlanes, pl.tmin, pl.cap, v.offsets, v.sorted, v.k0, ys));
    MSM_STAGE("big sort");
  } else {
    const dim3 pb(256), pgb((unsigned)((npts * batch + 255) / 256), NS);
    const unsigned ib = (unsigned)pl.iscan_blocks;
    msm_digits_kernel<FrP, 0><<<pgb, pb, 0, st>>>(sc, coef_d, plen, c, nwin, wide, pl.pre_stride, pl.pre_off, v.counts, nullptr,
                                                 nullptr, bid, v.canon, ys);
    MSM_STAGE("digits/count");
    iscan_block_kernel<<<dim3(ib, NS), dim3(ISCAN_THREADS), 0, st>>>(v.counts, nkeys, v.bt, nullptr, nullptr, nullptr, 0, ys);
    iscan_carry_kernel<<<dim3(1, NS), dim3(ISCAN_THREADS), 0, st>>>(v.bt, pl.iscan_blocks, ys);
    iscan_block_kernel<<<dim3(ib, NS), dim3(ISCAN_THREADS), 0, st>>>(v.counts, nkeys, nullptr, v.bt, v.offsets, v.cursor, 1, ys);
    MSM_STAGE("scan");
    msm_lane_start_kernel<<<dim3((pl.nlanes + 255) / 256, NS), dim3(256), 0, st>>>(v.offsets, (uint32_t)nkeys, pl.nlanes, pl.tmin,
                                                                                 pl.cap, v.k0, ys);
    msm_digits_kernel<FrP, 1><<<pgb, pb, 0, st>>>(sc, coef_d, plen, c, nwin, wide, pl.pre_stride, pl.pre_off, nullptr, v.cursor,
                                                 v.sorted, bid, v.canon, ys);
  }
  return ZK_OK;
}

template <class Fr, class Fld, class KF>
int msm_stage_accumulate(IEngine* eng, const MsmPlan& pl, const MsmViews<Fr, KF>& v, const MsmGate& gate, const void* bases,
                         const void* bases2, hipStream_t st) {
  constexpr bool G2FLD = IsExtField<Fld>::value;
  const unsigned NB = pl.vectors;
  const uint32_t nkeys = (uint32_t)pl.nkeys, nlanes = pl.nlanes;
  ProfScope ps_(eng->prof, G2FLD ? PROF_MSM_ACC_G2 : PROF_MSM_ACC_G1, st, (double)pl.npts * NB * pl.batch);
  if (gate.sorted_ev) {
    MSM_HIP(hipEventRecord(gate.sorted_ev, st));
    if (gate.sorted_cnt) gate.sorted_cnt->fetch_add(1, std::memory_order_release);
  }
  if (gate.n_wait_sorted) {
    if (!eng->spin_until([&] { return gate.sorted_cnt->load(std::memory_order_acquire) >= gate.sorted_need; }))
      return eng->fail(ZK_ERR_GENERIC, "msm launch: the sorts of the proof's other MSMs were not all enqueued within the deadline (" +
                                           std::to_string(gate.sorted_cnt->load()) + " of " + std::to_string(gate.sorted_need) + ")");
    for (int i = 0; i < gate.n_wait_sorted; i++) MSM_HIP(hipStreamWaitEvent(st, gate.wait_sorted[i], 0));
  }
  if (gate.wait_ev) {
    if (gate.wait_flag && !eng->spin_until([&] { return gate.wait_flag->load(std::memory_order_acquire) != 0; }))
      return eng->fail(ZK_ERR_GENERIC, "msm launch: the accumulate kernel ahead of this one in the batch's chain was not enqueued within the deadline");
    MSM_HIP(hipStreamWaitEvent(st, gate.wait_ev, 0));
  }
  if constexpr (G2FLD) {
    msm_accumulate_split_kernel<typename BaseParams<Fld>::type><<<dim3((nlanes + 31) / 32, NB), dim3(128), 0, st>>>(
        bases, bases2, v.sorted, v.offsets, nkeys, nlanes, pl.tmin, pl.cap, v.buckets, v.edge, v.heavy, v.k0, pl.ys);
  } else {
    msm_accumulate_kernel<KF><<<dim3((nlanes + 127) / 128, NB), dim3(128), 0, st>>>(
        (const Affine<KF>*)bases, (const Affine<KF>*)bases2, v.sorted, v.offsets, nkeys, nlanes, pl.tmin, pl.cap, v.buckets,
        v.edge, v.heavy, v.k0, pl.ys, 0);
  }
  if (gate.signal_ev) {
    MSM_HIP(hipEventRecord(gate.signal_ev, st));
    if (gate.signal_flag) gate.signal_flag->store(1, std::memory_order_release);
  }
  return ZK_OK;
}

template <class Fr, class Fld, class KF>
int msm_stage_reduce(IEngine* eng, const MsmPlan& pl, const MsmViews<Fr, KF>& v, hipStream_t st) {
  constexpr bool G2FLD = IsExtField<Fld>::value;
  const unsigned NB = pl.vectors, nsets = (unsigned)pl.nsets;
  const uint32_t nkeys = (uint32_t)pl.nkeys, nlanes = pl.nlanes, tmin = pl.tmin, cap = pl.cap;
  const size_t ys = pl.ys;
  ProfScope ps_(eng->prof, G2FLD ? PROF_MSM_REDUCE_G2 : PROF_MSM_REDUCE, st, (double)pl.nkeys * NB);
  const int qt = quad_threads(pl.batch > 1), qvl = qt / 4;
  const size_t quad_lds = (size_t)qvl * sizeof(XYZZ<Fld>);
  msm_heavy_kernel<KF><<<dim3(2048, NB), dim3(64), (size_t)16 * sizeof(XYZZ<Fld>), st>>>(v.edge, nlanes, tmin, cap, v.offsets, nkeys,
                                                                    v.buckets, v.heavy, v.hpart, pl.vcap, ys);
  MSM_STAGE("heavy buckets");
  {
    const size_t fin_wgs = std::min<size_t>((pl.nkeys + FIN_THREADS / 4 - 1) / (FIN_THREADS / 4), 8192);
    const unsigned fin_extra = 256;
    msm_finalize_kernel<KF><<<dim3((unsigned)fin_wgs + fin_extra, NB), dim3(FIN_THREADS),
                              (size_t)(FIN_THREADS / 4) * sizeof(XYZZ<Fld>), st>>>(
        v.edge, nlanes, tmin, cap, v.offsets, nkeys, v.buckets, v.heavy, v.hpart, pl.vcap, (uint32_t)fin_wgs, ys);
  }
  MSM_STAGE("finalize");
  const size_t tot_groups = (size_t)pl.red_groups * NB * nsets;
  const size_t tot_slices = (size_t)pl.nslices * NB * nsets;
  const size_t cap_quads = (size_t)1024 * (G2FLD ? 2 : 3) * 16;
  auto pick_nvl = [&](size_t groups) {
    int n = qvl;
    while (n > 4 && groups * (size_t)n > cap_quads) n >>= 1;
    return n;
  };
  const int nvl_a = pick_nvl(tot_groups), nvl_b = pick_nvl(tot_slices);
  const unsigned gpw_a = (unsigned)(qvl / nvl_a), gpw_b = (unsigned)(qvl / nvl_b);
  msm_reduce_a_kernel<KF><<<dim3((pl.red_groups + gpw_a - 1) / gpw_a, NB * nsets), dim3((unsigned)qt), quad_lds, st>>>(
      v.buckets, pl.B, pl.lo_bits, nvl_a, v.rc);
  msm_reduce_b_kernel<KF><<<dim3(((unsigned)pl.nslices + gpw_b - 1) / gpw_b, NB * nsets), dim3((unsigned)qt), quad_lds, st>>>(
      v.rc, pl.B, pl.lo_bits, nvl_b, v.out,
      v.offsets + nkeys, ys, pl.nsorts, v.stats);
  return ZK_OK;
}

template <class FrP, class Fld>
int msm_launch(IEngine* eng, MsmSlot& slot, const MsmTuning& tune, const void* bases, const void* bases2,
               const void* scalars, size_t npts, const Fp<FrP>* coef_d, size_t part_len, hipStream_t st,
               MsmPending* pend, const MsmBatchArg* ba) {
  using Fr = Fp<FrP>;
  using KF = typename KernelField<Fld>::type;
  static_assert(sizeof(KF) == sizeof(Fld), "kernel field layout");
  static_assert(sizeof(XYZZ<Fld>) == 4 * sizeof(Fld), "the plan sizes XYZZ points as four coordinates");
  constexpr bool G2FLD = IsExtField<Fld>::value;
  *pend = MsmPending{};
  const unsigned NB = bases2 ? 2u : 1u;
  const void* const bases_in = bases;
  const void* const bases2_in = bases2;
  size_t toff = 0, toff2 = 0;
  std::shared_ptr<const MsmTable> tab = TableRegistry::inst().find(bases, npts, sizeof(Affine<Fld>), FrP::BITS, &toff), tab2;
  if (tab && NB == 2) {
    tab2 = TableRegistry::inst().find(bases2, npts, sizeof(Affine<Fld>), FrP::BITS, &toff2);
    if (!tab2 || tab2->len != tab->len || toff2 != toff || tab2->c != tab->c) tab = nullptr;
    else bases2 = tab2->data;
  }
  if (tab) bases = tab->data;
  MsmPlanIn in;
  in.scalar_bits = FrP::BITS, in.scalar_bytes = (int)sizeof(Fr), in.coord_bytes = (int)sizeof(Fld), in.g2 = G2FLD;
  if constexpr (G2FLD) in.acc_waves = SPLIT_WAVES<typename BaseParams<Fld>::type>;
  else in.acc_waves = ACC_WAVES<Fld>;
  in.npts = npts, in.batch = ba ? (size_t)ba->nb : 1, in.vectors = (int)NB;
  if (tab) {
    in.tab_c = tab->c, in.tab_len = tab->len, in.tab_off = toff;
    in.tab_no_identity = !tab->any_identity && (NB == 1 || !tab2->any_identity);
  }
  in.c_force = tune.c_force, in.bigsort_min = tune.bigsort_min;
  const MsmPlan pl = msm_plan(in);
  if (pl.err) return eng->fail(ZK_ERR_BAD_INPUT, pl.err);
  pend->fold = pl.fold;
  if (npts == 0) return ZK_OK;
  hipError_t he = slot.ws.ensure(pl.ws_bytes);
  if (he != hipSuccess) return eng->hip_fail(he, "msm workspace");
  he = slot.ensure_pinned(pl.pinned_bytes);
  if (he != hipSuccess) return eng->hip_fail(he, "msm pinned buffer");
  if (!slot.ev) {
    he = hipEventCreateWithFlags(&slot.ev, hipEventDisableTiming);
    if (he != hipSuccess) return eng->hip_fail(he, "msm event");
  }
  slot.busy = true;
  slot.tab = tab;
  slot.tab2 = tab2;
  pend->slot = &slot;
  struct RecordOnExit {
    MsmSlot& s;
    hipStream_t st;
    bool done = false;
    ~RecordOnExit() {
      if (!done) (void)hipEventRecord(s.ev, st);
    }
  } record_on_exit{slot, st};
  const MsmViews<Fr, KF> v(pl, slot.ws.p, slot.pinned);
  MsmScalars<Fr> sc{};
  for (size_t b = 0; b < pl.batch; b++) sc.p[b] = (const Fr*)(ba ? ba->p[b] : scalars);
  sc.npts = (uint32_t)npts;
  sc.nb = (uint32_t)pl.batch;
  sc.sets_per = (uint32_t)pl.kwin;
  MsmBaseId bid;
  if (!pl.no_identity) {
    bid.b0 = bases_in;
    bid.b1 = bases2_in;
    bid.elem16 = (uint32_t)(sizeof(Affine<KF>) / 16);
  }
  int rc = msm_stage_sort<FrP, KF>(eng, pl, v, sc, coef_d, part_len ? part_len : npts, bid, st);
  if (rc) return rc;
  MSM_STAGE("scatter");
  rc = msm_stage_accumulate<Fr, Fld, KF>(eng, pl, v, tune.gate, bases, bases2, st);
  if (rc) return rc;
  MSM_STAGE("accumulate");
  rc = msm_stage_reduce<Fr, Fld, KF>(eng, pl, v, st);
  if (rc) return rc;
  MSM_HIP(hipGetLastError());
  MSM_STAGE("reduce");
  MSM_HIP(hipEventRecord(slot.ev, st));
  record_on_exit.done = true;
  return ZK_OK;
}
#undef MSM_HIP
#undef MSM_STAGE

template <class FrP, class Fld>
int msm_table_launch(IEngine* eng, const void* bases, size_t len, int c, int nwin, int wide, void* table,
                     hipStream_t st) {
  using KF = typename KernelField<Fld>::type;
  msm_table_kernel<KF><<<dim3((unsigned)((len + 127) / 128)), dim3(128), 0, st>>>(
      (const Affine<KF>*)bases, len, c, nwin, wide, (Affine<KF>*)table);
  hipError_t he = hipGetLastError();
  if (he != hipSuccess) return eng->hip_fail(he, "msm_table_kernel");
  return ZK_OK;
}

template <class FrP, class Fld>
int pack_points_split_launch(IEngine* eng, const void* points, size_t nchunks, int n, const uint8_t* dig, int jlen,
                             const void* beta, void* shares, hipStream_t st) {
  if constexpr (IsExtField<Fld>::value) {
    using P = typename BaseParams<Fld>::type;
    Fp<P> b;
    memcpy(&b, beta, sizeof(b));
    pss_pack_points_jsf_split_kernel<FrP, P><<<dim3((unsigned)((nchunks * 4 + 127) / 128), (unsigned)n), dim3(128), 0, st>>>(
        (const Affine<Fp2<P>>*)points, nchunks, n, dig, jlen, b, (Affine<Fp2<P>>*)shares);
    hipError_t he = hipGetLastError();
    if (he != hipSuccess) return eng->hip_fail(he, "pss_pack_points_jsf_split_kernel");
    return ZK_OK;
  } else {
    return eng->fail(ZK_ERR_BAD_INPUT, "the quad-split pack kernel is for extension-field points");
  }
}

template <class FrP, class Fld>
int base_mul_split_launch(IEngine* eng, const void* scalars, size_t len, const void* table, int nwin, int wb, void* out,
                          hipStream_t st) {
  if constexpr (IsExtField<Fld>::value) {
    using P = typename BaseParams<Fld>::type;
    const dim3 grid((unsigned)((len * 4 + 127) / 128)), block(128);
    if (wb == 16)
      fixed_base_mul_split_kernel<FrP, P, 16><<<grid, block, 0, st>>>((const Fp<FrP>*)scalars, len, (const Affine<Fp2<P>>*)table,
                                                                      nwin, (Affine<Fp2<P>>*)out);
    else
      fixed_base_mul_split_kernel<FrP, P, 8><<<grid, block, 0, st>>>((const Fp<FrP>*)scalars, len, (const Affine<Fp2<P>>*)table,
                                                                     nwin, (Affine<Fp2<P>>*)out);
    hipError_t he = hipGetLastError();
    if (he != hipSuccess) return eng->hip_fail(he, "fixed_base_mul_split_kernel");
    return ZK_OK;
  } else {
    return eng->fail(ZK_ERR_BAD_INPUT, "the quad-split fixed-base kernel is for extension-field points");
  }
}

#define ZK_INSTANTIATE_MSM(FRP, FLD)                                                                              \
  template int msm_launch<FRP, FLD>(IEngine*, MsmSlot&, const MsmTuning&, const void*, const void*, const void*, \
                                    size_t, const Fp<FRP>*, size_t, hipStream_t, MsmPending*, const MsmBatchArg*);  \
  template int msm_table_launch<FRP, FLD>(IEngine*, const void*, size_t, int, int, int, void*, hipStream_t);     \
  template int pack_points_split_launch<FRP, FLD>(IEngine*, const void*, size_t, int, const uint8_t*, int, const void*, void*, hipStream_t); \
  template int base_mul_split_launch<FRP, FLD>(IEngine*, const void*, size_t, const void*, int, int, void*, hipStream_t);

}
```

zk-saas_amd/csrc/quad.hpp:

```cpp
#pragma once
#include "ec.hpp"
#include "ntt.hpp"

namespace zk {
#if defined(__HIPCC__)

template <int P0, int P1, int P2, int P3>
ZK_D uint32_t qperm_u32(uint32_t v) {
  return (uint32_t)__builtin_amdgcn_mov_dpp((int)v, P0 | (P1 << 2) | (P2 << 4) | (P3 << 6), 0xf, 0xf, true);
}
template <int P0, int P1, int P2, int P3, class P>
ZK_D Fp<P> qperm(const Fp<P>& v) {
  Fp<P> r;
#pragma unroll
  for (int i = 0; i < P::N; i++) r.v[i] = qperm_u32<P0, P1, P2, P3>(v.v[i]);
  return r;
}
template <int P0, int P1, int P2, int P3, class P, bool I>
ZK_D Fp2T<P, I> qperm(const Fp2T<P, I>& v) {
  return {qperm<P0, P1, P2, P3>(v.c0), qperm<P0, P1, P2, P3>(v.c1)};
}
template <class P>
ZK_D Fp<P> qsel(bool a, const Fp<P>& x, const Fp<P>& y) {
  Fp<P> r;
// ... 76 lines not shown
  const Fp<P> ao = cswap(a);
  return (a + qsel(comp, a, ao)) * qsel(comp, ao, a - ao);
}
template <class P>
ZK_D bool s2_is_zero(const Fp<P>& a) {
  const uint32_t z = a.is_zero() ? 1u : 0u;
  return (z & qperm_u32<1, 0, 3, 2>(z)) != 0;
}
template <class P>
struct SplitAcc {
  Fp<P> c0, c1;
};
template <class P>
ZK_D SplitAcc<P> split_identity(bool comp) {
  return SplitAcc<P>{qsel(comp, Fp<P>::zero(), Fp<P>::one()), Fp<P>::zero()};
}
template <class P>
ZK_D SplitAcc<P> split_madd(const SplitAcc<P>& a, const Fp<P>& in, bool half, bool comp) {
  using F = Fp<P>;
  const uint32_t zz = s2_is_zero(a.c1) ? 1u : 0u;
  SplitAcc<P> r;
  if (qperm_u32<0, 0, 0, 0>(zz)) {
    r.c0 = in;
    r.c1 = qsel(comp, F::zero(), F::one());
    return r;
  }
  const F m1 = s2_mul(in, a.c1, comp);
  const F d = m1 - a.c0;
  const F od = hswap(d);
  const uint32_t dz = s2_is_zero(d) ? 1u : 0u;
  const bool pz = qperm_u32<0, 0, 0, 0>(dz) != 0, rz = qperm_u32<2, 2, 2, 2>(dz) != 0;
  if (pz) {
    if (!rz) return split_identity<P>(comp);
    const F u = qsel(half, in.dbl(), in);
    const F m2 = s2_sqr(u, comp);
    const F o2 = hswap(m2);
    const F m3 = s2_mul(u, qsel(half, m2, o2), comp);
    const F M = m2.dbl() + m2;
    const F m4 = s2_sqr(M, comp);
    const F X3 = m4 - m3.dbl();
    const F m5 = s2_mul(qsel(half, m3, M), qsel(half, in, m3 - X3), comp);
    const F o5 = hswap(m5);
    r.c0 = qsel(half, o5 - m5, X3);
    r.c1 = qsel(half, m3, o2);
    return r;
  }
  const F m2 = s2_sqr(d, comp);
  const F o2 = hswap(m2);
  const F m3 = s2_mul(qsel(half, od, a.c0), qsel(half, o2, m2), comp);
  const F o3 = hswap(m3);
  const F m4 = s2_mul(a.c1, qsel(half, m3, m2), comp);
  const F X3 = o2 - o3 - m3.dbl();
  const F m5 = s2_mul(qsel(half, a.c0, od), qsel(half, m3, m3 - X3), comp);
  const F o5 = hswap(m5);
  r.c0 = qsel(half, o5 - m5, X3);
  r.c1 = m4;
  return r;
}

template <class P>
ZK_D SplitAcc<P> split_dbl(const SplitAcc<P>& a, bool half, bool comp) {
  using F = Fp<P>;
  const uint32_t zz = s2_is_zero(a.c1) ? 1u : 0u;
  if (qperm_u32<0, 0, 0, 0>(zz)) return a;
  const F u = qsel(half, a.c0.dbl(), a.c0);
  const F m1 = s2_sqr(u, comp);
  const F o1 = hswap(m1);
  const F m2 = s2_mul(u, qsel(half, m1, o1), comp);
  const F M = m1.dbl() + m1;
  const F m3 = s2_mul(qsel(half, m2, M), qsel(half, a.c0, M), comp);
  const F X3 = m3 - m2.dbl();
  const F m4 = s2_mul(qsel(half, m2, M), qsel(half, a.c1, m2 - X3), comp);
  const F m5 = s2_mul(o1, a.c1, comp);
  SplitAcc<P> r;
  r.c0 = qsel(half, hswap(m4) - m3, X3);
  r.c1 = qsel(half, m4, m5);
  return r;
}

template <class P>
ZK_D Fp<P> split_inv(const Fp<P>& z, bool comp) {
  const Fp<P> sq = z * z;
  const Fp<P> ninv = (sq + cswap(sq)).inverse_fast();
  const Fp<P> r = z * ninv;
  return qsel(comp, r.neg(), r);
}
ZK_D bool quad_all(bool b) {
  uint32_t z = b ? 1u : 0u;
  z &= qperm_u32<1, 0, 3, 2>(z);
  z &= qperm_u32<2, 3, 0, 1>(z);
  return z != 0;
}
template <class P>
__device__ __noinline__ Fp<P> split_affine_add(const Fp<P>& a, bool ida, const Fp<P>& b, bool idb, bool half, bool comp,
                                               bool* idr) {
  using F = Fp<P>;
  *idr = false;
  if (ida) {
    *idr = idb;
    return b;
  }
  if (idb) return a;
  const F d = b - a;
  const uint32_t dz = s2_is_zero(d) ? 1u : 0u;
  const bool xz = qperm_u32<0, 0, 0, 0>(dz) != 0, yz = qperm_u32<2, 2, 2, 2>(dz) != 0;
  const F xa = qperm<0, 1, 0, 1>(a), ya = qperm<2, 3, 2, 3>(a);
  F lam;
  if (xz) {
    if (!yz) {
      *idr = true;
      return F::zero();
    }
    const F xx = s2_sqr(xa, comp);
    lam = s2_mul(xx.dbl() + xx, split_inv(ya.dbl(), comp), comp);
  } else {
    lam = s2_mul(qperm<2, 3, 2, 3>(d), split_inv(qperm<0, 1, 0, 1>(d), comp), comp);
  }
  const F x3 = s2_sqr(lam, comp) - xa - qperm<0, 1, 0, 1>(b);
  const F y3 = s2_mul(lam, xa - x3, comp) - ya;
  return qsel(half, y3, x3);
}

template <class P>
ZK_D void split_store_affine(const SplitAcc<P>& acc, Fp<P>* dst, bool half, bool comp) {
  using F = Fp<P>;
  const uint32_t zz = s2_is_zero(acc.c1) ? 1u : 0u;
  if (qperm_u32<0, 0, 0, 0>(zz)) {
    store_elem(dst, F::zero());
    return;
  }
  const F zi = split_inv(qperm<2, 3, 2, 3>(acc.c1), comp);
  const F zi2 = s2_sqr(s2_mul(zi, qperm<0, 1, 0, 1>(acc.c1), comp), comp);
  store_elem(dst, s2_mul(acc.c0, qsel(half, zi, zi2), comp));
}

template <class Fld>
ZK_D Fld wg_quad_sum(Fld c, XYZZ<Fld>* sh, int vl, int q, int nvl) {
  qstore(sh + vl, q, c);
  __syncthreads();
  for (int off = nvl >> 1; off >= 1; off >>= 1) {
    const bool act = (vl & (nvl - 1)) < off;
    Fld r = c;
    if (act) r = qadd(c, qload(sh + vl + off, q), q);
    __syncthreads();
    if (act) {
      c = r;
      qstore(sh + vl, q, c);
    }
    __syncthreads();
  }
  return c;
}

#endif
}
```

Baseline: 647.0 proofs/s.

## Use 8-lane octet point addition for G2 MSM tail kernels

```diff
diff --git a/include/zksaas.h b/include/zksaas.h
--- a/include/zksaas.h
+++ b/include/zksaas.h
@@ -48,6 +48,7 @@
 int zk_fft1(zk_ctx* ctx, void* shares_d, int log2_m, int inverse, size_t batch, const void* add_d, void* stream);
 int zk_fq_selftest(zk_ctx* ctx, int op, const void* a_d, const void* b_d, const void* c_d, const void* d_d, size_t len,
                    void* out_d, void* stream);
+int zk_oadd_selftest(zk_ctx* ctx, const void* a_d, const void* b_d, size_t len, void* out_d, void* stream);
 int zk_fft2_king(zk_ctx* ctx, const void* in_d, const uint32_t* parties, int nparties, int log2_m, int inverse,
                  const void* g, int scale_size_inv, int rearrange, uint64_t seed, void* out_d,
                  const void* out_mask_d, void* stream);
diff --git a/rust/zksaas-hip-sys/src/lib.rs b/rust/zksaas-hip-sys/src/lib.rs
--- a/rust/zksaas-hip-sys/src/lib.rs
+++ b/rust/zksaas-hip-sys/src/lib.rs
@@ -166,6 +166,14 @@
         out_d: *mut c_void,
         stream: *mut c_void,
     ) -> c_int;
+    pub fn zk_oadd_selftest(
+        ctx: *mut ZkCtx,
+        a_d: *const c_void,
+        b_d: *const c_void,
+        len: usize,
+        out_d: *mut c_void,
+        stream: *mut c_void,
+    ) -> c_int;
     pub fn zk_fft2_king(
         ctx: *mut ZkCtx,
         in_d: *const c_void,
diff --git a/zk-saas_amd/_lib.py b/zk-saas_amd/_lib.py
--- a/zk-saas_amd/_lib.py
+++ b/zk-saas_amd/_lib.py
@@ -19,7 +19,7 @@
     "zk_points_decompress", "zk_points_compress", "zk_libsnark_h", "zk_vec_scale", "zk_deg_red_parties", "zk_d_msm_parties", "zk_pss_pack_points", "zk_msm_plan",
     "zk_msm_mask_sample", "zk_r1cs_qap", "zk_fr_to_bytes", "zk_fr_from_bytes", "zk_ctx_set_option", "zk_msm_precompute", "zk_msm_forget", "zk_msm_table_info",
     "zk_groth16_prove_batch", "zk_groth16_prove_batch_async", "zk_groth16_batch_wait", "zk_msm_batch", "zk_pss_unpack_points", "zk_pss_unpack2_points", "zk_groth16_reconstruct", "zk_msm_stats", "zk_dist_groth16_prove_batch", "zk_d_fft_host", "zk_msm_host", "zk_d_msm_host",
-    "zk_net_parties", "zk_dist_groth16_prove_async", "zk_dist_groth16_wait", "zk_fq_selftest",
+    "zk_net_parties", "zk_dist_groth16_prove_async", "zk_dist_groth16_wait", "zk_fq_selftest", "zk_oadd_selftest",
     "zk_dist_deg_red_points", "zk_dist_libsnark_h", "zk_deg_red_host", "zk_d_pp_host", "zk_circom_h_host",
     "zk_groth16_prove_host",
 ]
@@ -150,6 +150,7 @@
     lib.zk_dist_circom_h.argtypes = [vp, vp, vp, vp, vp, i32, vp, u64, vp, vp]
     lib.zk_dist_groth16_prove.argtypes = [vp, vp, vp, vp, vp, vp, vp, vp, vp, vp, i32, vp, u64, vp, vp, vp, vp]
     lib.zk_fq_selftest.argtypes = [vp, i32, vp, vp, vp, vp, sz, vp, vp]
+    lib.zk_oadd_selftest.argtypes = [vp, vp, vp, sz, vp, vp]
     lib.zk_net_parties.argtypes = [vp, i32, C.POINTER(i32)]
     lib.zk_dist_groth16_prove_async.argtypes = [vp, vp, vp, vp, vp, vp, vp, vp, vp, vp, i32, vp, u64, vp, C.POINTER(i32)]
     lib.zk_dist_groth16_wait.argtypes = [vp, vp, i32, vp, vp, vp]
diff --git a/zk-saas_amd/csrc/api.cpp b/zk-saas_amd/csrc/api.cpp
--- a/zk-saas_amd/csrc/api.cpp
+++ b/zk-saas_amd/csrc/api.cpp
@@ -168,6 +168,10 @@
   CTX_OR_FAIL();
   return e->fq_selftest(op, a_d, b_d, c_d, d_d, len, out_d, S(stream));
 }
+int zk_oadd_selftest(zk_ctx* ctx, const void* a_d, const void* b_d, size_t len, void* out_d, void* stream) {
+  CTX_OR_FAIL();
+  return e->oadd_selftest(a_d, b_d, len, out_d, S(stream));
+}
 
 int zk_fft1(zk_ctx* ctx, void* shares_d, int log2_m, int inverse, size_t batch, const void* add_d, void* stream) {
   CTX_OR_FAIL();
diff --git a/zk-saas_amd/csrc/engine.hpp b/zk-saas_amd/csrc/engine.hpp
--- a/zk-saas_amd/csrc/engine.hpp
+++ b/zk-saas_amd/csrc/engine.hpp
@@ -248,6 +248,7 @@
   virtual int vec_mul_sub(void* out, const void* a, const void* b, const void* c, size_t len, hipStream_t st) = 0;
   virtual int fq_selftest(int op, const void* a, const void* b, const void* c, const void* d, size_t len, void* out,
                           hipStream_t st) = 0;
+  virtual int oadd_selftest(const void* a, const void* b, size_t len, void* out, hipStream_t st) = 0;
   virtual int fft1(void* shares, int log_m, int inverse, size_t batch, const void* add, hipStream_t st) = 0;
   virtual int fft2_king(const void* in, const void* in_mask, const uint32_t* parties, int np, int log_m, int inverse,
                         const void* g, int scale_size_inv, int rearrange, uint64_t seed, void* out,
diff --git a/zk-saas_amd/csrc/engine_fft.inc.hpp b/zk-saas_amd/csrc/engine_fft.inc.hpp
--- a/zk-saas_amd/csrc/engine_fft.inc.hpp
+++ b/zk-saas_amd/csrc/engine_fft.inc.hpp
@@ -95,6 +95,12 @@
         op, (const Fq*)a, (const Fq*)b, (const Fq*)c, (const Fq*)d, len, (Fq*)out);
     ZK_HIP(hipGetLastError());
     return ZK_OK;
+  }
+  int oadd_selftest(const void* a, const void* b, size_t len, void* out, hipStream_t st) override {
+    if (!len) return ZK_OK;
+    if (!a || !b || !out) return fail(ZK_ERR_BAD_INPUT, "null pointer");
+    if constexpr (Cfg::HAS_G2) return oadd_selftest_launch<FrP, Fp2<typename Cfg::FqP>>(this, a, b, len, out, st);
+    else return fail(ZK_ERR_BAD_INPUT, "G2 is not available for this curve");
   }
 
   int fft1(void* shares, int log_m, int inverse, size_t batch, const void* add, hipStream_t st) override {
diff --git a/zk-saas_amd/csrc/msm.hpp b/zk-saas_amd/csrc/msm.hpp
--- a/zk-saas_amd/csrc/msm.hpp
+++ b/zk-saas_amd/csrc/msm.hpp
@@ -1012,9 +1012,14 @@
 inline int quad_threads(bool batched) {
   return batched ? 64 : 256;
 }
-
 template <class Fld>
-__global__ __launch_bounds__(64) void msm_heavy_kernel(const XYZZ<Fld>* __restrict__ edge0, uint32_t nlanes, uint32_t tmin,
+constexpr int TAIL_WAVES_1W = IsExtField<Fld>::value ? tail_waves<Fld>() : 0;
+template <class Fld>
+constexpr int TAIL_WAVES_RED = IsExtField<Fld>::value ? tail_waves<Fld>() : 2;
+
+template <class Fld>
+__global__ __launch_bounds__(64, TAIL_WAVES_1W<Fld>)
+void msm_heavy_kernel(const XYZZ<Fld>* __restrict__ edge0, uint32_t nlanes, uint32_t tmin,
                                                        uint32_t cap, const uint32_t* __restrict__ offsets, uint32_t nkeys,
                                                        XYZZ<Fld>* __restrict__ buckets0,
                                                        const uint32_t* __restrict__ heavy,
@@ -1031,8 +1036,10 @@
   extern __shared__ uint4 smem_fin[];
   XYZZ<Fld>* sh = reinterpret_cast<XYZZ<Fld>*>(smem_fin);
   const uint32_t T = msm_range_len(offsets[nkeys], nlanes, tmin, cap);
-  const int q = threadIdx.x & 3, vl = threadIdx.x >> 2;
-  const int nq = (int)blockDim.x / 4;
+  using G = LaneGroup<Fld>;
+  using Lane = typename G::Lane;
+  const int q = threadIdx.x & (G::W - 1), vl = threadIdx.x / G::W;
+  const int nq = (int)blockDim.x / G::W;
   for (uint32_t v = blockIdx.x; v < V; v += gridDim.x) {
     uint32_t lo = 0, hi = nh;
     while (hi - lo > 1) {
@@ -1046,17 +1053,18 @@
     const uint32_t l0 = o0 / T, l1 = (o1 - 1) / T;
     const uint32_t chunk = (l1 - l0 + S - 1) / S;
     const uint32_t first = l0 + 1 + s * chunk, last = first + chunk - 1 < l1 ? first + chunk - 1 : l1;
-    Fld acc = (s == 0 && vl == 0) ? qload(tail + l0, q) : qidentity<Fld>(q);
-    for (uint32_t l = first + (uint32_t)vl; l <= last; l += (uint32_t)nq) acc = qadd(acc, qload(head + l, q), q);
-    acc = wg_quad_sum(acc, sh, vl, q, nq);
-    if (vl == 0) qstore(S == 1 ? buckets + kh : hpart + v, q, acc);
+    Lane acc = (s == 0 && vl == 0) ? G::load(tail + l0, q) : G::identity(q);
+    for (uint32_t l = first + (uint32_t)vl; l <= last; l += (uint32_t)nq) acc = G::add(acc, G::load(head + l, q), q);
+    acc = G::wg_sum(acc, sh, vl, q, nq);
+    if (vl == 0) G::store(S == 1 ? buckets + kh : hpart + v, q, acc);
     __syncthreads();
   }
 }
 
 constexpr int FIN_THREADS = 64;
 template <class Fld>
-__global__ __launch_bounds__(FIN_THREADS) void msm_finalize_kernel(const XYZZ<Fld>* __restrict__ edge0, uint32_t nlanes,
+__global__ __launch_bounds__(FIN_THREADS, TAIL_WAVES_1W<Fld>)
+void msm_finalize_kernel(const XYZZ<Fld>* __restrict__ edge0, uint32_t nlanes,
                                                                uint32_t tmin, uint32_t cap,
                                                                const uint32_t* __restrict__ offsets, uint32_t nkeys,
                                                                XYZZ<Fld>* __restrict__ buckets0,
@@ -1068,43 +1076,47 @@
   const XYZZ<Fld>* __restrict__ head = edge0 + (size_t)blockIdx.y * 2 * nlanes;
   const XYZZ<Fld>* __restrict__ tail = head + nlanes;
   XYZZ<Fld>* __restrict__ buckets = buckets0 + (size_t)blockIdx.y * nkeys;
-  const int q = threadIdx.x & 3;
+  using G = LaneGroup<Fld>;
+  using Lane = typename G::Lane;
+  constexpr int FIN_VL = FIN_THREADS / G::W;
+  const int q = threadIdx.x & (G::W - 1);
   if (blockIdx.x >= fin_wgs) {
     ZK_YSHIFT(heavy);
     const uint32_t nh = heavy[1], V = heavy[0];
     const XYZZ<Fld>* __restrict__ hpart = hpart0 + (size_t)blockIdx.y * vcap;
     extern __shared__ uint4 smem_fin[];
     XYZZ<Fld>* sh = reinterpret_cast<XYZZ<Fld>*>(smem_fin);
-    const int vl = threadIdx.x >> 2;
+    const int vl = threadIdx.x / G::W;
     for (uint32_t h = blockIdx.x - fin_wgs; h < nh; h += gridDim.x - fin_wgs) {
       const uint32_t vb = heavy[3 + 2 * h], S = (h + 1 < nh ? heavy[3 + 2 * (h + 1)] : V) - vb;
       if (S == 1) continue;
-      Fld acc = qidentity<Fld>(q);
-      for (uint32_t j = (uint32_t)vl; j < S; j += FIN_THREADS / 4) acc = qadd(acc, qload(hpart + vb + j, q), q);
-      acc = wg_quad_sum(acc, sh, vl, q, FIN_THREADS / 4);
-      if (vl == 0) qstore(buckets + heavy[2 + 2 * h], q, acc);
+      Lane acc = G::identity(q);
+      for (uint32_t j = (uint32_t)vl; j < S; j += FIN_VL) acc = G::add(acc, G::load(hpart + vb + j, q), q);
+      acc = G::wg_sum(acc, sh, vl, q, FIN_VL);
+      if (vl == 0) G::store(buckets + heavy[2 + 2 * h], q, acc);
       __syncthreads();
     }
     return;
   }
   const uint32_t T = msm_range_len(offsets[nkeys], nlanes, tmin, cap);
-  for (size_t k = (size_t)blockIdx.x * (FIN_THREADS / 4) + (threadIdx.x >> 2); k < nkeys;
-       k += (size_t)fin_wgs * (FIN_THREADS / 4)) {
+  for (size_t k = (size_t)blockIdx.x * FIN_VL + threadIdx.x / G::W; k < nkeys;
+       k += (size_t)fin_wgs * FIN_VL) {
     const uint32_t o0 = offsets[k], o1 = offsets[k + 1];
     if (o0 == o1) {
-      qstore(buckets + k, q, qidentity<Fld>(q));
+      G::store(buckets + k, q, G::identity(q));
       continue;
     }
     const uint32_t l0 = o0 / T, l1 = (o1 - 1) / T;
     if (l1 == l0 || l1 - l0 > FIN_SEQ) continue;
-    Fld acc = qload(tail + l0, q);
-    for (uint32_t l = l0 + 1; l <= l1; l++) acc = qadd(acc, qload(head + l, q), q);
-    qstore(buckets + k, q, acc);
+    Lane acc = G::load(tail + l0, q);
+    for (uint32_t l = l0 + 1; l <= l1; l++) acc = G::add(acc, G::load(head + l, q), q);
+    G::store(buckets + k, q, acc);
   }
 }
 
 template <class Fld>
-__global__ __launch_bounds__(QUAD_THREADS, 2) void msm_reduce_a_kernel(const XYZZ<Fld>* __restrict__ buckets0, uint32_t B,
+__global__ __launch_bounds__(QUAD_THREADS, TAIL_WAVES_RED<Fld>)
+void msm_reduce_a_kernel(const XYZZ<Fld>* __restrict__ buckets0, uint32_t B,
                                                                    int lo_bits, int nvl, XYZZ<Fld>* __restrict__ out0) {
   __builtin_amdgcn_s_setprio(3);
   extern __shared__ uint4 smem_red[];
@@ -1112,28 +1124,31 @@
   const uint32_t LO = 1u << lo_bits, HI = B >> lo_bits;
   const uint32_t ngroups = HI + 1 + LO;
   const XYZZ<Fld>* __restrict__ wb = buckets0 + (size_t)blockIdx.y * B;
-  const int q = threadIdx.x & 3, vl = threadIdx.x >> 2;
-  const uint32_t g = blockIdx.x * (uint32_t)((int)blockDim.x / 4 / nvl) + (uint32_t)(vl / nvl);
+  using G = LaneGroup<Fld>;
+  using Lane = typename G::Lane;
+  const int q = threadIdx.x & (G::W - 1), vl = threadIdx.x / G::W;
+  const uint32_t g = blockIdx.x * (uint32_t)((int)blockDim.x / G::W / nvl) + (uint32_t)(vl / nvl);
   const uint32_t sub = (uint32_t)(vl & (nvl - 1));
-  Fld acc = qidentity<Fld>(q);
+  Lane acc = G::identity(q);
   if (g <= HI) {
     for (uint32_t lo = sub; lo < LO; lo += (uint32_t)nvl) {
       uint32_t k = g * LO + lo;
-      if (k >= 1 && k <= B) acc = qadd(acc, qload(wb + (k - 1), q), q);
+      if (k >= 1 && k <= B) acc = G::add(acc, G::load(wb + (k - 1), q), q);
     }
   } else if (g < ngroups) {
     const uint32_t lo = g - HI - 1;
     for (uint32_t hi = sub; hi <= HI; hi += (uint32_t)nvl) {
       uint32_t k = hi * LO + lo;
-      if (k >= 1 && k <= B) acc = qadd(acc, qload(wb + (k - 1), q), q);
-    }
-  }
-  acc = wg_quad_sum(acc, sh, vl, q, nvl);
-  if (sub == 0 && g < ngroups) qstore(out0 + (size_t)blockIdx.y * ngroups + g, q, acc);
+      if (k >= 1 && k <= B) acc = G::add(acc, G::load(wb + (k - 1), q), q);
+    }
+  }
+  acc = G::wg_sum(acc, sh, vl, q, nvl);
+  if (sub == 0 && g < ngroups) G::store(out0 + (size_t)blockIdx.y * ngroups + g, q, acc);
 }
 
 template <class Fld>
-__global__ __launch_bounds__(QUAD_THREADS, 2) void msm_reduce_b_kernel(const XYZZ<Fld>* __restrict__ rc0, uint32_t B, int lo_bits,
+__global__ __launch_bounds__(QUAD_THREADS, TAIL_WAVES_RED<Fld>)
+void msm_reduce_b_kernel(const XYZZ<Fld>* __restrict__ rc0, uint32_t B, int lo_bits,
                                                                    int nvl, XYZZ<Fld>* __restrict__ out0,
                                                                    const uint32_t* __restrict__ cnt_src, size_t cnt_stride,
                                                                    uint32_t ncnt, uint32_t* __restrict__ cnt_dst) {
@@ -1148,20 +1163,33 @@
   while ((1u << hb) < HI) hb++;
   const int nslices = hb + 1 + lo_bits;
   const XYZZ<Fld>* __restrict__ rc = rc0 + (size_t)blockIdx.y * ngroups;
-  const int q = threadIdx.x & 3, vl = threadIdx.x >> 2;
-  const int j = (int)blockIdx.x * ((int)blockDim.x / 4 / nvl) + vl / nvl;
+  using G = LaneGroup<Fld>;
+  using Lane = typename G::Lane;
+  const int q = threadIdx.x & (G::W - 1), vl = threadIdx.x / G::W;
+  const int j = (int)blockIdx.x * ((int)blockDim.x / G::W / nvl) + vl / nvl;
   const uint32_t sub = (uint32_t)(vl & (nvl - 1));
-  Fld acc = qidentity<Fld>(q);
+  Lane acc = G::identity(q);
   if (j <= hb) {
     for (uint32_t hi = sub; hi <= HI; hi += (uint32_t)nvl)
-      if ((hi >> j) & 1u) acc = qadd(acc, qload(rc + hi, q), q);
+      if ((hi >> j) & 1u) acc = G::add(acc, G::load(rc + hi, q), q);
   } else if (j < nslices) {
     const int jj = j - hb - 1;
     for (uint32_t lo = sub; lo < LO; lo += (uint32_t)nvl)
-      if ((lo >> jj) & 1u) acc = qadd(acc, qload(rc + HI + 1 + lo, q), q);
-  }
-  acc = wg_quad_sum(acc, sh, vl, q, nvl);
-  if (sub == 0 && j < nslices) qstore(out0 + (size_t)blockIdx.y * nslices + j, q, acc);
+      if ((lo >> jj) & 1u) acc = G::add(acc, G::load(rc + HI + 1 + lo, q), q);
+  }
+  acc = G::wg_sum(acc, sh, vl, q, nvl);
+  if (sub == 0 && j < nslices) G::store(out0 + (size_t)blockIdx.y * nslices + j, q, acc);
+}
+
+template <class Fld>
+__global__ __launch_bounds__(64, TAIL_WAVES_1W<Fld>) void oadd_selftest_kernel(const XYZZ<Fld>* __restrict__ a,
+                                                                             const XYZZ<Fld>* __restrict__ b, size_t len,
+                                                                             XYZZ<Fld>* __restrict__ out) {
+  using G = LaneGroup<Fld>;
+  const int o = threadIdx.x & (G::W - 1);
+  const size_t i = (size_t)blockIdx.x * (64 / G::W) + threadIdx.x / G::W;
+  if (i >= len) return;
+  G::store(out + i, o, G::add(G::load(a + i, o), G::load(b + i, o), o));
 }
 
 template <class Fld>
@@ -1267,6 +1295,8 @@
 template <class FrP, class Fld>
 int base_mul_split_launch(IEngine* eng, const void* scalars, size_t len, const void* table, int nwin, int wb, void* out,
                           hipStream_t st);
+template <class FrP, class Fld>
+int oadd_selftest_launch(IEngine* eng, const void* a, const void* b, size_t len, void* out, hipStream_t st);
 template <class FrP, class Fld>
 int msm_table_launch(IEngine* eng, const void* bases, size_t len, int c, int nwin, int wide, void* table,
                      hipStream_t st);
diff --git a/zk-saas_amd/csrc/msm_impl.hpp b/zk-saas_amd/csrc/msm_impl.hpp
--- a/zk-saas_amd/csrc/msm_impl.hpp
+++ b/zk-saas_amd/csrc/msm_impl.hpp
@@ -157,22 +157,23 @@
   const uint32_t nkeys = (uint32_t)pl.nkeys, nlanes = pl.nlanes, tmin = pl.tmin, cap = pl.cap;
   const size_t ys = pl.ys;
   ProfScope ps_(eng->prof, G2FLD ? PROF_MSM_REDUCE_G2 : PROF_MSM_REDUCE, st, (double)pl.nkeys * NB);
-  const int qt = quad_threads(pl.batch > 1), qvl = qt / 4;
+  constexpr int GW = tail_lanes<Fld>();
+  const int qt = quad_threads(pl.batch > 1), qvl = qt / GW;
   const size_t quad_lds = (size_t)qvl * sizeof(XYZZ<Fld>);
-  msm_heavy_kernel<KF><<<dim3(2048, NB), dim3(64), (size_t)16 * sizeof(XYZZ<Fld>), st>>>(v.edge, nlanes, tmin, cap, v.offsets, nkeys,
-                                                                    v.buckets, v.heavy, v.hpart, pl.vcap, ys);
+  msm_heavy_kernel<KF><<<dim3(2048, NB), dim3(64), (size_t)(64 / GW) * sizeof(XYZZ<Fld>), st>>>(
+      v.edge, nlanes, tmin, cap, v.offsets, nkeys, v.buckets, v.heavy, v.hpart, pl.vcap, ys);
   MSM_STAGE("heavy buckets");
   {
-    const size_t fin_wgs = std::min<size_t>((pl.nkeys + FIN_THREADS / 4 - 1) / (FIN_THREADS / 4), 8192);
+    const size_t fin_wgs = std::min<size_t>((pl.nkeys + FIN_THREADS / GW - 1) / (FIN_THREADS / GW), 8192);
     const unsigned fin_extra = 256;
     msm_finalize_kernel<KF><<<dim3((unsigned)fin_wgs + fin_extra, NB), dim3(FIN_THREADS),
-                              (size_t)(FIN_THREADS / 4) * sizeof(XYZZ<Fld>), st>>>(
+                              (size_t)(FIN_THREADS / GW) * sizeof(XYZZ<Fld>), st>>>(
         v.edge, nlanes, tmin, cap, v.offsets, nkeys, v.buckets, v.heavy, v.hpart, pl.vcap, (uint32_t)fin_wgs, ys);
   }
   MSM_STAGE("finalize");
   const size_t tot_groups = (size_t)pl.red_groups * NB * nsets;
   const size_t tot_slices = (size_t)pl.nslices * NB * nsets;
-  const size_t cap_quads = (size_t)1024 * (G2FLD ? 2 : 3) * 16;
+  const size_t cap_quads = (size_t)1024 * (G2FLD ? tail_waves<Fld>() : 3) * (64 / GW);
   auto pick_nvl = [&](size_t groups) {
     int n = qvl;
     while (n > 4 && groups * (size_t)n > cap_quads) n >>= 1;
@@ -320,11 +321,27 @@
   }
 }
 
+template <class FrP, class Fld>
+int oadd_selftest_launch(IEngine* eng, const void* a, const void* b, size_t len, void* out, hipStream_t st) {
+  if constexpr (IsExtField<Fld>::value) {
+    using KF = typename KernelField<Fld>::type;
+    constexpr size_t per_wg = 64 / tail_lanes<Fld>();
+    oadd_selftest_kernel<KF><<<dim3((unsigned)((len + per_wg - 1) / per_wg)), dim3(64), 0, st>>>(
+        (const XYZZ<KF>*)a, (const XYZZ<KF>*)b, len, (XYZZ<KF>*)out);
+    hipError_t he = hipGetLastError();
+    if (he != hipSuccess) return eng->hip_fail(he, "oadd_selftest_kernel");
+    return ZK_OK;
+  } else {
+    return eng->fail(ZK_ERR_BAD_INPUT, "the octet addition is for extension-field points");
+  }
+}
+
 #define ZK_INSTANTIATE_MSM(FRP, FLD)                                                                              \
   template int msm_launch<FRP, FLD>(IEngine*, MsmSlot&, const MsmTuning&, const void*, const void*, const void*, \
                                     size_t, const Fp<FRP>*, size_t, hipStream_t, MsmPending*, const MsmBatchArg*);  \
   template int msm_table_launch<FRP, FLD>(IEngine*, const void*, size_t, int, int, int, void*, hipStream_t);     \
   template int pack_points_split_launch<FRP, FLD>(IEngine*, const void*, size_t, int, const uint8_t*, int, const void*, void*, hipStream_t); \
-  template int base_mul_split_launch<FRP, FLD>(IEngine*, const void*, size_t, const void*, int, int, void*, hipStream_t);
-
-}
+  template int base_mul_split_launch<FRP, FLD>(IEngine*, const void*, size_t, const void*, int, int, void*, hipStream_t);   \
+  template int oadd_selftest_launch<FRP, FLD>(IEngine*, const void*, const void*, size_t, void*, hipStream_t);
+
+}
diff --git a/zk-saas_amd/csrc/quad.hpp b/zk-saas_amd/csrc/quad.hpp
--- a/zk-saas_amd/csrc/quad.hpp
+++ b/zk-saas_amd/csrc/quad.hpp
@@ -252,5 +252,135 @@
   return c;
 }
 
+ZK_D int olane_base() { return (int)(threadIdx.x & 56u); }
+template <int P0, int P1, int P2, int P3>
+ZK_D uint32_t operm_u32(uint32_t v, int o) {
+  if constexpr (P0 < 2 && P1 < 2 && P2 >= 2 && P3 >= 2 && (P0 & 1) == (P2 & 1) && (P1 & 1) == (P3 & 1)) {
+    return qperm_u32<(P0 & 1) * 2, (P0 & 1) * 2 + 1, (P1 & 1) * 2, (P1 & 1) * 2 + 1>(v);
+  } else {
+    const int src = ((P0 | (P1 << 2) | (P2 << 4) | (P3 << 6)) >> (o & 6)) & 3;
+    return (uint32_t)__builtin_amdgcn_ds_bpermute((olane_base() | (src << 1) | (o & 1)) << 2, (int)v);
+  }
+}
+template <int P0, int P1, int P2, int P3, class P>
+ZK_D Fp<P> operm(const Fp<P>& v, int o) {
+  Fp<P> r;
+#pragma unroll
+  for (int i = 0; i < P::N; i++) r.v[i] = operm_u32<P0, P1, P2, P3>(v.v[i], o);
+  return r;
+}
+template <int K>
+ZK_D bool ozero(uint64_t zmask) {
+  return ((uint32_t)(zmask >> (olane_base() + 2 * K)) & 3u) == 3u;
+}
+template <class P>
+ZK_D uint64_t ozmask(const Fp<P>& v) {
+  return __ballot(v.is_zero() ? 1 : 0);
+}
+template <class P>
+ZK_D Fp<P> oidentity(int o) {
+  return qsel(o == 0 || o == 2, Fp<P>::one(), Fp<P>::zero());
+}
+template <class P, bool I>
+ZK_D Fp<P> oload(const XYZZ<Fp2T<P, I>>* p, int o) {
+  return load_elem(reinterpret_cast<const Fp<P>*>(p) + o);
+}
+template <class P, bool I>
+ZK_D void ostore(XYZZ<Fp2T<P, I>>* p, int o, const Fp<P>& c) {
+  store_elem(reinterpret_cast<Fp<P>*>(p) + o, c);
+}
+
+template <class P>
+ZK_D Fp<P> oadd(const Fp<P>& ca_in, const Fp<P>& cb, int o) {
+  using F = Fp<P>;
+  const int k = o >> 1;
+  const bool comp = (o & 1) != 0, even = (k & 1) == 0;
+  const bool za = ozero<2>(ozmask(ca_in)), zb = ozero<2>(ozmask(cb));
+  const bool idn = za || zb;
+  const F ca = qsel(za, cb, ca_in);
+  const F zza = operm<2, 2, 3, 3>(ca, o), zzb = operm<2, 2, 3, 3>(cb, o);
+  F A = qsel(even, operm<0, 0, 1, 1>(ca, o), operm<0, 0, 1, 1>(cb, o));
+  F B = qsel(even, zzb, zza);
+  const F m1 = s2_mul(A, B, comp);
+  const F d = operm<1, 1, 3, 3>(m1, o) - operm<0, 0, 2, 2>(m1, o);
+  const uint64_t dz = ozmask(d);
+  const bool pz = ozero<0>(dz), rz = ozero<2>(dz);
+  const bool D = pz && rz && !idn;
+  const F cu = qsel(k == 1, ca.dbl(), ca);
+  A = qsel(D, cu, qsel(even, d, zza));
+  B = qsel(D, cu, qsel(even, d, zzb));
+  const F m2 = s2_mul(A, B, comp);
+  const F XX = operm<0, 0, 0, 0>(m2, o);
+  const F m2_1 = operm<1, 1, 1, 1>(m2, o);
+  const F M = XX.dbl() + XX;
+  A = qsel(D, qsel(k == 3, M, cu), qsel(k == 2, m2_1, qsel(k == 1, d, m1)));
+  B = qsel(D, qsel(k == 3, M, m2_1), XX);
+  const F m3 = s2_mul(A, B, comp);
+  const F m3_1 = operm<1, 1, 1, 1>(m3, o);
+  const F m3_0 = operm<0, 0, 0, 0>(m3, o);
+  const F T = qsel(D, operm<3, 3, 3, 3>(m3, o), operm<2, 2, 2, 2>(m2, o)) - m3_0.dbl();
+  const F X3f = qsel(D, T, T - m3_1);
+  A = qsel(D, qsel(k == 0, M, m3_1),
+           qsel(k == 1, operm<2, 2, 2, 2>(d, o), qsel(k == 0, operm<2, 2, 2, 2>(m1, o), m2)));
+  B = qsel(D, qsel(k == 0, m3_0 - X3f, ca),
+           qsel(k == 1, m3_0 - X3f, m3_1));
+  const F m4 = s2_mul(A, B, comp);
+  const F m4_0 = operm<0, 0, 0, 0>(m4, o), m4_1 = operm<1, 1, 1, 1>(m4, o);
+  const F Y3 = qsel(D, m4_0 - m4_1, m4_1 - m4_0);
+  F r = qsel(k == 0, X3f, qsel(k == 1, Y3, qsel(k == 2, m3, m4)));
+  if (pz && !rz) r = oidentity<P>(o);
+  if (idn) r = ca;
+  return r;
+}
+
+template <class P, bool I>
+ZK_D Fp<P> wg_octet_sum(Fp<P> c, XYZZ<Fp2T<P, I>>* sh, int vl, int o, int nvl) {
+  ostore(sh + vl, o, c);
+  __syncthreads();
+  for (int off = nvl >> 1; off >= 1; off >>= 1) {
+    const bool act = (vl & (nvl - 1)) < off;
+    Fp<P> r = c;
+    if (act) r = oadd(c, oload(sh + vl + off, o), o);
+    __syncthreads();
+    if (act) {
+      c = r;
+      ostore(sh + vl, o, c);
+    }
+    __syncthreads();
+  }
+  return c;
+}
+
+template <class Fld>
+struct LaneGroup {
+  static constexpr int W = 4;
+  using Lane = Fld;
+  static ZK_D Lane identity(int q) { return qidentity<Fld>(q); }
+  static ZK_D Lane load(const XYZZ<Fld>* p, int q) { return qload(p, q); }
+  static ZK_D void store(XYZZ<Fld>* p, int q, const Lane& c) { qstore(p, q, c); }
+  static ZK_D Lane add(const Lane& a, const Lane& b, int q) { return qadd(a, b, q); }
+  static ZK_D Lane wg_sum(const Lane& c, XYZZ<Fld>* sh, int vl, int q, int nvl) { return wg_quad_sum(c, sh, vl, q, nvl); }
+};
+template <class P, bool I>
+struct LaneGroup<Fp2T<P, I>> {
+  static constexpr int W = 8;
+  using Fld = Fp2T<P, I>;
+  using Lane = Fp<P>;
+  static ZK_D Lane identity(int o) { return oidentity<P>(o); }
+  static ZK_D Lane load(const XYZZ<Fld>* p, int o) { return oload(p, o); }
+  static ZK_D void store(XYZZ<Fld>* p, int o, const Lane& c) { ostore(p, o, c); }
+  static ZK_D Lane add(const Lane& a, const Lane& b, int o) { return oadd(a, b, o); }
+  static ZK_D Lane wg_sum(const Lane& c, XYZZ<Fld>* sh, int vl, int o, int nvl) { return wg_octet_sum(c, sh, vl, o, nvl); }
+};
+
 #endif
-}
+
+template <class Fld>
+constexpr int tail_lanes() {
+  return IsExtField<Fld>::value ? 8 : 4;
+}
+template <class Fld>
+constexpr int tail_waves() {
+  return sizeof(Fld) > 64 ? 2 : 4;
+}
+}
```

After: 663.5 proofs/s (median of 6 runs). 1.03x the previous value.
